# cmbant/getdist

Hardware: AMD Instinct MI355X
Metric: 2D KDE densities/sec (triangle, 50 params, 1e+07 samples) (higher is better)
Workload: dtype f64

## Files before the change

getdist_amd/_lib.py:

```python

import ctypes as C
import os
import subprocess

import numpy as np

_HERE = os.path.dirname(os.path.abspath(__file__))
LIB_PATH = os.path.join(_HERE, "csrc", "libgdhip.so")

GD_OK, GD_ERR_BADARG, GD_ERR_NOMEM, GD_ERR_HIP, GD_ERR_EMPTY, GD_ERR_SOLVER, GD_ERR_FFT, GD_ERR_NODEVICE, GD_ERR_TIMEOUT = \
    0, -1, -2, -3, -4, -5, -6, -7, -8


class GdhipError(RuntimeError):
    def __init__(self, code, msg):
        super().__init__("libgdhip error %d: %s" % (code, msg))
        self.code = code


class GdhipTimeout(GdhipError):
    """GD_ERR_TIMEOUT: a collective or the communicator set-up gave up waiting for a peer; the library has aborted and dropped
    the communicator, so the ranks renegotiate over the host application's own channel (parallel.init_library_comm)."""


def build_native(force=False):
    script = os.path.join(_HERE, "csrc", "build.sh")
    if force:
        for f in os.listdir(os.path.join(_HERE, "csrc")):
            if f.endswith(".o") or f.endswith(".so"):
                os.remove(os.path.join(_HERE, "csrc", f))
    subprocess.run(["bash", script], check=True)
    return LIB_PATH


_p = C.c_void_p
_i32, _i64, _f64 = C.c_int32, C.c_int64, C.c_double
_pd = C.POINTER(C.c_double)
_pi32 = C.POINTER(C.c_int32)
_pi64 = C.POINTER(C.c_int64)

SIGNATURES = {
    "gd_device_count": (C.c_int, []),
    "gd_create": (C.c_int, [C.c_int, C.POINTER(_p)]),
    "gd_destroy": (None, [_p]),
    "gd_last_error": (C.c_char_p, [_p]),
    "gd_version": (C.c_char_p, []),
    "gd_device_info": (C.c_int, [_p, _pi64]),
    "gd_sync": (C.c_int, [_p]),
    "gd_dev_alloc": (C.c_int, [_p, _i64, C.POINTER(_p)]),
    "gd_dev_free": (C.c_int, [_p, _p]),
    "gd_memcpy_h2d": (C.c_int, [_p, _p, _p, _i64]),
    "gd_memcpy_d2h": (C.c_int, [_p, _p, _p, _i64]),
    "gd_memcpy_d2h_async": (C.c_int, [_p, _p, _p, _i64]),
    "gd_copy_sync": (C.c_int, [_p]),
    "gd_memcpy_d2d": (C.c_int, [_p, _p, _p, _i64]),
    "gd_memset": (C.c_int, [_p, _p, C.c_int, _i64]),
    "gd_gather_items": (C.c_int, [_p, _p, _p, _pi32, _i32, _i64]),
    "gd_host_alloc": (C.c_int, [_p, _i64, C.POINTER(_p)]),
    "gd_host_free": (C.c_int, [_p, _p]),
    "gd_kde_lag_sums_2d": (C.c_int, [_p, _i32, _i32, _pd, _pi64, _i32, _pd]),
    "gd_autocov_lags_batch": (C.c_int, [_p, _pi32, _i32, _pd, _i64, _i32, _pd]),
    "gd_kde_lag_sums_batch": (C.c_int, [_p, _pi32, _i32, _pd, _pi64, _i32, _pd]),
    "gd_autocov_lags_range_batch": (C.c_int, [_p, _pi32, _i32, _pd, _i64, _i64, _i64, _i32, _pd]),
    "gd_timer_start": (C.c_int, [_p]),
    "gd_timer_stop_ms": (C.c_int, [_p, _pd]),
    "gd_upload": (C.c_int, [_p, _p, _i64, _i64, _i64, _i64, _p]),
    "gd_num_rows": (C.c_int, [_p, _pi64, _pi64]),
    "gd_column_ptr": (C.c_int, [_p, _i64, C.POINTER(_p)]),
    "gd_weight_stats": (C.c_int, [_p, _i64, _i64, _f64, _pd]),
    "gd_col_stats": (C.c_int, [_p, _i64, _i64, _pd]),
    "gd_cov": (C.c_int, [_p, _pi32, _i32, _i64, _i64, _pd, _pd, _pd, _pd]),
    "gd_quantiles": (C.c_int, [_p, _pi32, _i32, _i64, _i64, _pd, _i32, _pd]),
    "gd_quantiles_mm_probe": (C.c_int, [_p, _pi32, _i32, _i64, _i64, _pd, _i32, _pd, _pd, _pd, _pd, C.POINTER(C.c_int32)]),
    "gd_quantiles_mm": (C.c_int, [_p, _pi32, _i32, _i64, _i64, _pd, _i32, _pd, _pd]),
    "gd_autocov_lags": (C.c_int, [_p, _i32, _f64, _i64, _i32, _pd]),
    "gd_kde_lag_sums": (C.c_int, [_p, _i32, _f64, _pi64, _i32, _pd]),
    "gd_hist1d": (C.c_int, [_p, _pi32, _i32, _pd, _pd, _i32, _pd]),
    "gd_hist1d_dev": (C.c_int, [_p, _pi32, _i32, _pd, _pd, _i32, _p]),
    "gd_bin_indices": (C.c_int, [_p, _i32, _f64, _f64, _i32, _i32, _pi32, _pi64]),
    "gd_prebin": (C.c_int, [_p, _i32, _f64, _f64, _i32, _p]),
    "gd_prebin_batch": (C.c_int, [_p, _pi32, _i32, _pd, _pd, _i32, C.POINTER(_p)]),
    "gd_prebin8_batch": (C.c_int, [_p, _pi32, _i32, _pd, _pd, _i32, C.POINTER(_p), _pi64]),
    "gd_hist2d_prebinned8": (C.c_int, [_p, _i32, C.POINTER(_p), C.POINTER(_p), _p]),
    "gd_prebin8_hist2d": (C.c_int, [_p, _pi32, _i32, _pd, _pd, C.POINTER(_p), _pi64, _i32, C.POINTER(_p), C.POINTER(_p), _p]),
    "gd_hist2d": (C.c_int, [_p, _i32, _pi32, _pi32, _pd, _pd, _pd, _pd, _i32, _p]),
    "gd_hist2d_prebinned": (C.c_int, [_p, _i32, C.POINTER(_p), C.POINTER(_p), _i32, _p]),
    "gd_minmax_affine": (C.c_int, [_p, _i32, _pi32, _pi32, _pd, _pd, _pd]),
    "gd_hist2d_sheared": (C.c_int, [_p, _i32, _pi32, _pi32, _pd, _pd, _pd, _pd, _pd, _pd, _i32, _p]),
    "gd_dct1d": (C.c_int, [_p, _i32, _i32, _pd, _pd]),
    "gd_isj1d": (C.c_int, [_p, _i32, _i32, _pd, _pd, _pd, _pi32]),
    "gd_isj1d_dev": (C.c_int, [_p, _i32, _i32, _p, _pd, _pd, _pi32]),
    "gd_density1d": (C.c_int, [_p, _i32, _i32, _pd, _pd, _pi32, _pi32, _i32, _i32, _pd, _pi32]),
    "gd_density1d_dev": (C.c_int, [_p, _i32, _i32, _p, _pd, _pi32, _pi32, _i32, _i32, _pd, _pi32]),
    "gd_density1d_batch": (C.c_int, [_p, _p, _p, _i32, _pi32, _i32, _pd, _pd, _pd]),
    "gd_kopt2d": (C.c_int, [_p, _i32, _i32, _p, _pd, _pi32, _pd, _pd, _pd]),
    "gd_kopt2d_enqueue": (C.c_int, [_p, _i32, _i32, _p, _pd, _pi32, _pd, _pd, _p, _pi32]),
    "gd_kopt2d_finish": (C.c_int, [_p, _p, _i32, _i32, _p, _pd]),
    "gd_get_h": (C.c_int, [_p, _i32, _pd, _pd, _pd, _pi32, _pd]),
    "gd_density2d": (C.c_int, [_p, _i32, _i32, _p, _pd, _pd, _pd, _pi32, _pi32, _i32, _i32, _p, _pi32]),
    "gd_copy_mark": (C.c_int, [_p, _pi32]),
    "gd_copy_wait": (C.c_int, [_p, _i32]),
    "gd_density2d_enqueue": (C.c_int, [_p, _i32, _i32, _p, _pd, _pd, _pd, _pi32, _pi32, _i32, _i32, _p, _p]),
    "gd_density2d_enqueue_indexed": (C.c_int, [_p, _i32, _i32, _p, _pi32, _pd, _pd, _pd, _pi32, _pi32, _i32, _i32, _p, _p]),
    "gd_attach_samples": (C.c_int, [_p, _p]),
    "gd_bind_thread": (C.c_int, [_p]),
    "gd_contour_levels": (C.c_int, [_p, _i32, _i32, _p, _pd, _i32, _pd, _pi32]),
    "gd_limits1d": (C.c_int, [_p, _i32, _i32, _pd, _pd, _pd, _pd, _i32, _i32, _pd, _pi32]),
    "gd_set_extra_column": (C.c_int, [_p, _i32, _pd]),
    "gd_aux_weights": (C.c_int, [_p, _pd]),
    "gd_col_minmax": (C.c_int, [_p, _pi32, _i32, _i64, _i64, _i32, C.c_double, _pd]),
    "gd_weights_integral": (C.c_int, [_p, _pi32]),
    "gd_thin_rows": (C.c_int, [_p, _i64, _i64, _i64, _i32, _p, _i64, C.POINTER(C.c_int64)]),
    "gd_binary_transitions": (C.c_int, [_p, _pi32, _i32, _p, _i64, _pd, _i32, C.POINTER(C.c_int64)]),
    "gd_thinned_lag_sums": (C.c_int, [_p, _pi32, _i32, _pd, _p, _i64, _i32, _pd]),
    "gd_density2d_masked": (C.c_int, [_p, _i32, _p, C.c_double, C.c_double, C.c_double, _i32, _i32, _i32, _i32, _pd, _pd,
                                      C.POINTER(C.c_ubyte), _p, _pi32]),
    "gd_like_weights": (C.c_int, [_p, _pd, _i32, C.c_double, _pd]),
    "gd_select_weights": (C.c_int, [_p, _i32]),
    "gd_likes1d": (C.c_int, [_p, _i32, _i32, _pd, _pd, _pd, _pd, _pi32, _pi32, _i32, _pd, _pi32]),
    "gd_likes2d": (C.c_int, [_p, _i32, _i32, _p, _p, _pd, _pd, _pd, _pi32, _pi32, _i32, _p, _pi32]),
    "gd_circ_convolve": (C.c_int, [_p, _i32, _i32, _pd, _pd, _pd]),
    "gd_convolve1d_direct": (C.c_int, [_p, _pd, _i64, _pd, _i64, _pd]),
    "gd_autoconvolve": (C.c_int, [_p, _i32, _f64, _i32, _pd, _i64, _i64, _i64, _i32, _pd]),
    "gd_like_stats": (C.c_int, [_p, _i32, _pd]),
    "gd_batch2d_grid_sizes": (C.c_int, [_p, _i32, _pd, _pi32, _i32, _pi32]),
    "gd_density2d_batch": (C.c_int, [_p, _p, _p, _p, _i32, _pd, _pd, _pd, _pi32, _i32, _p, _p, _p, _i64, _pi32, _pd, _pd, _pi32,
                                     _pi32]),
    "gd_comm_unique_id": (C.c_int, [_p]),
    "gd_comm_init": (C.c_int, [_p, _i32, _i32, _p]),
    "gd_comm_info": (C.c_int, [_p, _pi32, _pi32]),
    "gd_comm_destroy": (C.c_int, [_p]),
    "gd_comm_abandon": (C.c_int, [_p]),
    "gd_comm_allgather": (C.c_int, [_p, _pd, _i64, _pd]),
    "gd_comm_allreduce_sum": (C.c_int, [_p, _pd, _i64]),
    "gd_comm_allgather_dev": (C.c_int, [_p, _p, _i64, _p]),
    "gd_comm_allreduce_sum_dev": (C.c_int, [_p, _p, _i64, _p]),
    "gd_batch2d_finish": (C.c_int, [_p]),
    "gd_batch2d_invalidate": (C.c_int, [_p]),
    "gd_batch2d_exchanges": (C.c_int, [_p, C.POINTER(C.c_int64)]),
    "gd_comm_rccl_path": (C.c_int, [C.c_char_p, C.c_int32, C.POINTER(C.c_int32)]),
    "gd_upload_shard": (C.c_int, [_p, _p, _i64, _i64, _i64, _i64, _i64, _p]),
    "gd_comm_share_columns": (C.c_int, [_p, C.POINTER(C.c_int64)]),
    "gd_histnd_batch": (C.c_int, [_p, _i32, _pi32, _pi32, _pd, _pd, _i32, _i32, _i32, _pd, _pd, _pd]),
    "gd_pca_corr": (C.c_int, [_p, _pi32, _i32, _pi32, _pd, _pd, _pd]),
    "gd_pca_project": (C.c_int, [_p, _pi32, _i32, _pi32, _pd, _pd, _pd, _i32, _i32, _pd, _pd, _pd, _pd, _pd, _pd]),
    "gd_mixture_nll": (C.c_int, [_p, _pi32, _i32, _i32, _pd, _pd, _pd, _i64, _i64, _pd]),
}

GD_HISTND_MAXD, GD_HISTND_MAX_BINS = 25, 1 << 25
GD_HISTND_H, GD_HISTND_LIKES, GD_HISTND_LMIN = 1, 2, 4
GD_PCA_MAX_PROJ = 448

_lib = None


def load_library():
    global _lib
    if _lib is None:
        if not os.path.exists(LIB_PATH):
            raise ImportError("libgdhip.so is not built: run `python -c 'import __graft_entry__ as g; g.build()'` "
                              "or getdist_amd/csrc/build.sh (there is no CPU fallback)")
        lib = C.CDLL(LIB_PATH)
        for name, (res, args) in SIGNATURES.items():
            fn = getattr(lib, name)
            fn.restype = res
            fn.argtypes = args
        _lib = lib
    return _lib


def _dp(a):
    return a.ctypes.data_as(_pd)


def _ip(a):
    return a.ctypes.data_as(_pi32)


def _f64arr(a):
    return np.ascontiguousarray(a, dtype=np.float64)


def _i32arr(a):
    return np.ascontiguousarray(a, dtype=np.int32)


class DevBuf:

    def __init__(self, ctx, nbytes):
        self.ctx = ctx
        self.nbytes = int(nbytes)
        self.ptr, self.capacity = ctx._take_block(self.nbytes)

    def free(self):
        if self.ptr and self.ctx.h:
            self.ctx._give_block(self.ptr, self.capacity)
        self.ptr = None

    def __del__(self):
        try:
            self.free()
        except Exception:
            pass

    def to_host(self, shape, dtype=np.float64, offset_bytes=0, pinned=False):
        out = self.ctx.pinned_array(shape, dtype) if pinned else np.empty(shape, dtype=dtype)
        self.ctx._check(self.ctx.lib.gd_memcpy_d2h(self.ctx.h, out.ctypes.data, self.ptr + offset_bytes, out.nbytes))
        return out

    def to_host_async(self, shape, dtype=np.float64):
        out = self.ctx.pinned_array(shape, dtype)
        self.ctx._check(self.ctx.lib.gd_memcpy_d2h_async(self.ctx.h, out.ctypes.data, self.ptr, out.nbytes))
        return out

    def from_host(self, arr, offset_bytes=0):
        arr = np.ascontiguousarray(arr)
        self.ctx._check(self.ctx.lib.gd_memcpy_h2d(self.ctx.h, self.ptr + offset_bytes, arr.ctypes.data, arr.nbytes))


class Context:

    def __init__(self, device=0):
        self.lib = load_library()
        self.h = None
        if self.lib.gd_device_count() <= 0:
            raise RuntimeError("getdist_amd needs a HIP device (no CPU fallback): none visible")
        h = _p()
        rc = self.lib.gd_create(int(device), C.byref(h))
        if rc != 0:
            raise GdhipError(rc, "gd_create(device=%d) failed" % device)
        self.h = h
        self.device = device
        self.N = self.n = 0
        self.weighted = False
        self._pinned = []
        self._free_blocks = []
        self._pinned_blocks = []
        self.comm_world = self.comm_rank = 0

    PINNED_POOL_LIMIT = 8 << 30

    def pinned_array(self, shape, dtype=np.float64):
        import sys

        nbytes = int(np.prod(shape)) * np.dtype(dtype).itemsize
        best = None
        for k, (ptr, nb, buf) in enumerate(self._pinned):
            if nb >= nbytes and sys.getrefcount(buf) <= 3 and (best is None or nb < self._pinned[best][1]):
                best = k
        if best is None:
# ... 482 lines not shown
                                                   thresholds.shape[1], out.ctypes.data_as(C.POINTER(C.c_int64))))
        return out

    def thinned_lag_sums(self, cols, means, rows, K, maxoff):
        cols, means = _i32arr(cols), _f64arr(means)
        out = np.zeros((len(cols), int(maxoff)))
        self._check(self.lib.gd_thinned_lag_sums(self.h, _ip(cols), len(cols), _dp(means), rows.ptr, int(K), int(maxoff),
                                                 _dp(out)))
        return out

    def like_weights(self, loglikes, mode, mean_loglike):
        if loglikes is None:
            self._check(self.lib.gd_like_weights(self.h, None, 0, 0.0, None))
            return None
        ll = _f64arr(loglikes)
        if ll.shape != (self.N,):
            raise ValueError("loglikes must have one entry per sample row")
        tot = C.c_double()
        self._check(self.lib.gd_like_weights(self.h, _dp(ll), int(mode), float(mean_loglike), C.byref(tot)))
        return tot.value

    def select_weights(self, which):
        self._check(self.lib.gd_select_weights(self.h, int(which)))

    def likes1d(self, hist, likehist, P, smooth, winw, flags, shade_mean_loglikes):
        hist, likehist, P = _f64arr(hist), _f64arr(likehist), _f64arr(P)
        B, F = hist.shape
        smooth, winw, flags = _f64arr(smooth), _i32arr(winw), _i32arr(flags)
        out = np.zeros_like(hist)
        status = np.zeros(B, dtype=np.int32)
        self._check(self.lib.gd_likes1d(self.h, B, F, _dp(hist), _dp(likehist), _dp(P), _dp(smooth), _ip(winw),
                                        _ip(flags), int(bool(shade_mean_loglikes)), _dp(out), _ip(status)))
        return out, status

    def likes2d(self, d_hist, d_likehist, B, F, rx, ry, corr, winw, flags, mbc):
        out = self.alloc(B * F * F * 8)
        rx, ry, corr, winw, flags = _f64arr(rx), _f64arr(ry), _f64arr(corr), _i32arr(winw), _i32arr(flags)
        status = np.zeros(B, dtype=np.int32)
        self._check(self.lib.gd_likes2d(self.h, B, F, d_hist.ptr, d_likehist.ptr, _dp(rx), _dp(ry), _dp(corr),
                                        _ip(winw), _ip(flags), int(mbc), out.ptr, _ip(status)))
        return out, status

    def circ_convolve(self, a, b):
        a, b = _f64arr(a), _f64arr(b)
        if a.shape != b.shape or a.ndim not in (1, 2):
            raise ValueError("circ_convolve needs two arrays of one shape, one- or two-dimensional")
        n0, n1 = (1, a.shape[0]) if a.ndim == 1 else a.shape
        out = np.empty_like(a)
        self._check(self.lib.gd_circ_convolve(self.h, int(n0), int(n1), _dp(a), _dp(b), _dp(out)))
        return out

    def convolve1d_direct(self, x, y):
        x, y = _f64arr(x), _f64arr(y)
        out = np.empty(x.size + y.size - 1)
        self._check(self.lib.gd_convolve1d_direct(self.h, _dp(x), x.size, _dp(y), y.size, _dp(out)))
        return out

    def autoconvolve(self, s, n, normalize=True, x=None, col=-1, mean=0.0, use_weights=False):
        out = np.empty(int(n))
        xx = None if x is None else _f64arr(x)
        self._check(self.lib.gd_autoconvolve(self.h, int(col), float(mean), int(bool(use_weights)),
                                             None if xx is None else _dp(xx), 0 if xx is None else xx.size, int(s), int(n),
                                             int(bool(normalize)), _dp(out)))
        return out

    def like_stats(self, col):
        out = np.zeros(8)
        self._check(self.lib.gd_like_stats(self.h, int(col), _dp(out)))
        return dict(min=out[0], max=out[1], norm=out[2], sum_wl=out[3], sum_wl2=out[4], sum_w_exp_plus=out[5],
                    sum_w_exp_minus=out[6], argmin=int(out[7]))

    def batch2d_grid_sizes(self, settings, n, corr, pairs32):
        F = np.zeros(len(pairs32), dtype=np.int32)
        rc = self.lib.gd_batch2d_grid_sizes(C.byref(settings), int(n), _dp(corr), _ip(pairs32), len(pairs32), _ip(F))
        if rc != 0:
            raise GdhipError(rc, "gd_batch2d_grid_sizes: bad argument")
        return F

    def density2d_batch(self, twin, settings, params, n, corr, cov, lag_probe, pairs32, exchange, grids, status, meta, levels,
                        level_status):
        tokens = np.full(2, -1, dtype=np.int32)
        self._check(self.lib.gd_density2d_batch(
            self.h, None if twin is None else twin.h, C.byref(settings), C.cast(params, _p), int(n), _dp(corr), _dp(cov),
            None if lag_probe is None else _dp(lag_probe), _ip(pairs32), len(pairs32),
            None if exchange is None else C.cast(exchange, _p), None, grids.ctypes.data, int(grids.size),
            status.ctypes.data_as(_pi32), _dp(meta), None if levels is None else _dp(levels),
            None if level_status is None else _ip(level_status), _ip(tokens)))
        return int(tokens[0]), int(tokens[1])

    @staticmethod
    def comm_unique_id():
        buf = C.create_string_buffer(128)
        rc = load_library().gd_comm_unique_id(buf)
        if rc != 0:
            raise GdhipError(rc, "gd_comm_unique_id failed (librccl.so missing?)")
        return buf.raw

    def comm_init(self, world, rank, id128):
        self._check(self.lib.gd_comm_init(self.h, int(world), int(rank), C.create_string_buffer(bytes(id128), 128)))
        self.comm_world, self.comm_rank = int(world), int(rank)

    def comm_allgather(self, vec):
        v = _f64arr(vec).ravel()
        out = np.empty((self.comm_world, v.size))
        self._check(self.lib.gd_comm_allgather(self.h, _dp(v), v.size, _dp(out)))
        return out

    def comm_allreduce_sum(self, vec):
        v = _f64arr(vec).ravel().copy()
        self._check(self.lib.gd_comm_allreduce_sum(self.h, _dp(v), v.size))
        return v

    def comm_destroy(self):
        self._check(self.lib.gd_comm_destroy(self.h))
        self.comm_world = 0

    def comm_info(self):
        wd, rk = C.c_int32(0), C.c_int32(0)
        self._check(self.lib.gd_comm_info(self.h, C.byref(wd), C.byref(rk)))
        return int(wd.value), int(rk.value)

    def comm_abandon(self):
        if self.h is not None:
            self.lib.gd_comm_abandon(self.h)

    def density1d_batch(self, settings, params, n, cols32, want_hist=False):
        cols32 = _i32arr(cols32)
        B, F = len(cols32), int(settings.fine_bins)
        P = np.zeros((B, F))
        hist = np.zeros((B, F)) if want_hist else None
        meta = np.zeros((B, 9))
        self._check(self.lib.gd_density1d_batch(self.h, C.byref(settings), C.cast(params, _p), int(n), _ip(cols32), B, _dp(P),
                                                None if hist is None else _dp(hist), _dp(meta)))
        return P, hist, meta

    def batch2d_finish(self):
        self._check(self.lib.gd_batch2d_finish(self.h))

    def batch2d_invalidate(self):
        self._check(self.lib.gd_batch2d_invalidate(self.h))

    def batch2d_exchanges(self):
        c = C.c_int64(0)
        self._check(self.lib.gd_batch2d_exchanges(self.h, C.byref(c)))
        return int(c.value)

    def kopt2d(self, d_hist, B, F, neff, do_corr, fallback_t, corr):
        neff, do_corr, fallback_t, corr = _f64arr(neff), _i32arr(do_corr), _f64arr(fallback_t), _f64arr(corr)
        out = np.zeros((B, 12))
        self._check(self.lib.gd_kopt2d(self.h, B, F, d_hist.ptr if isinstance(d_hist, DevBuf) else d_hist, _dp(neff),
                                       _ip(do_corr), _dp(fallback_t), _dp(corr), _dp(out)))
        return out

    def get_h(self, psi, neff, corr, do_corr):
        psi, neff, corr, do_corr = _f64arr(psi).reshape(-1, 6), _f64arr(neff), _f64arr(corr), _i32arr(do_corr)
        out = np.zeros((len(psi), 4))
        self._check(self.lib.gd_get_h(self.h, len(psi), _dp(psi), _dp(neff), _dp(corr), _ip(do_corr), _dp(out)))
        return out

    def density2d(self, d_hist, B, F, rx, ry, corr, winw, flags, bco, mbc, out=None):
        out = out or self.alloc(B * F * F * 8)
        rx, ry, corr, winw, flags = _f64arr(rx), _f64arr(ry), _f64arr(corr), _i32arr(winw), _i32arr(flags)
        status = np.zeros(B, dtype=np.int32)
        self._check(self.lib.gd_density2d(self.h, B, F, d_hist.ptr if isinstance(d_hist, DevBuf) else d_hist, _dp(rx),
                                          _dp(ry), _dp(corr), _ip(winw), _ip(flags), int(bco), int(mbc), out.ptr,
                                          _ip(status)))
        return out, status
```

getdist_amd/csrc/batch2d.hip:

```cpp
#include "batch1d.hpp"
#include "batch2d.hpp"
#include "ctx.hpp"

namespace {

gd_ctx* C(void* h) { return (gd_ctx*)h; }

const gdb::Ops kOps = {
     [](void* h) { return gd_bind_thread(C(h)); },
     [](void* h, int64_t* N, int64_t* n) { return gd_num_rows(C(h), N, n); },
    [](void* h, int32_t* hw) {
        gd_ctx* c = C(h);
        *hw = c->w == nullptr ? 0 : ((!c->w8 && !c->w_integral && c->w_sum > 1e-200 && c->w_sum < 1e200) ? 2 : 1);
        return 0;
    },
     [](void* h, int64_t bytes, void** out) { return gd_dev_alloc(C(h), bytes, out); },
     [](void* h, void* p) { return gd_dev_free(C(h), p); },
    [](void* h, const int32_t* cols, int32_t ncols, const double* binmin, const double* width, int32_t F, void* const* d_idx,
       int64_t* bad) { return gd_prebin8_batch(C(h), cols, ncols, binmin, width, F, d_idx, bad); },
    [](void* h, int32_t B, const void* const* ix, const void* const* iy, void* d_hist) {
        return gd_hist2d_prebinned8(C(h), B, ix, iy, d_hist);
    },
    [](void* h, const int32_t* cols, int32_t ncols, const double* binmin, const double* width, void* const* d_idx, int64_t* bad,
       int32_t B, const void* const* ix, const void* const* iy, void* d_hist) {
        return gd_prebin8_hist2d(C(h), cols, ncols, binmin, width, d_idx, bad, B, ix, iy, d_hist);
    },
    [](void* h, int32_t col, double binmin, double width, int32_t F, void* d_idx) {
        return gd_prebin(C(h), col, binmin, width, F, d_idx);
    },
    [](void* h, int32_t B, const void* const* ix, const void* const* iy, int32_t F, void* d_hist) {
        return gd_hist2d_prebinned(C(h), B, ix, iy, F, d_hist);
    },
    [](void* h, int32_t B, const int32_t* ci, const int32_t* cj, const double* a, const double* b, double* out) {
        return gd_minmax_affine(C(h), B, ci, cj, a, b, out);
    },
    [](void* h, int32_t B, const int32_t* ci, const int32_t* cj, const double* r0, const double* r1, const double* xmin,
       const double* dx, const double* ymin, const double* dy, int32_t F, void* d_hist) {
        return gd_hist2d_sheared(C(h), B, ci, cj, r0, r1, xmin, dx, ymin, dy, F, d_hist);
    },
    [](void* h, int32_t B, int32_t F, const void* d_hist, const double* neff, const int32_t* do_corr, const double* fallback_t,
       const double* corr, double* out) { return gd_kopt2d(C(h), B, F, d_hist, neff, do_corr, fallback_t, corr, out); },
    [](void* h, void* d_dst, int64_t dst_first, const void* d_src, const int32_t* index, int32_t count, int64_t item_bytes) {
        return gd_gather_items(C(h), (char*)d_dst + dst_first * item_bytes, d_src, index, count, item_bytes);
    },
    [](void* h, int32_t B, int32_t F, const void* d_hist, const int32_t* hist_index, const double* rx, const double* ry,
       const double* corr, const int32_t* winw, const int32_t* flags, int32_t bco, int32_t mbc, void* d_P, int32_t* status_pinned) {
        return gd_density2d_enqueue_indexed(C(h), B, F, d_hist, hist_index, rx, ry, corr, winw, flags, bco, mbc, d_P, status_pinned);
    },
     [](void* h, void* dst, const void* d_src, int64_t bytes) { return gd_memcpy_d2h_async(C(h), dst, d_src, bytes); },
     [](void* h, int32_t* token) { return gd_copy_mark(C(h), token); },
    [](void* h, int32_t token) {
        if (!gd_ctx_alive(C(h))) return 0;
        const int rc = gd_copy_wait(C(h), token);
        return rc == GD_ERR_BADARG ? 0 : rc;
    },
     [](void* h) { return gd_ctx_alive(C(h)) ? gd_copy_sync(C(h)) : 0; },
    [](void* h, int32_t B, int32_t F, const void* d_P, const double* contours, int32_t nc, double* out, int32_t* status) {
        return gd_contour_levels(C(h), B, F, d_P, contours, nc, out, status);
    },
    [](void* h, const int32_t* cols, int32_t ncols, const double* means, int64_t k0, int32_t nlags, double* out) {
        return gd_autocov_lags_batch(C(h), cols, ncols, means, k0, nlags, out);
    },
    [](void* h, const int32_t* cols, int32_t ncols, const double* inv4s2, const int64_t* lags, int32_t nlags, double* out) {
        return gd_kde_lag_sums_batch(C(h), cols, ncols, inv4s2, lags, nlags, out);
    },
    [](void* h, int32_t col, double inv4s2, const int64_t* lags, int32_t nlags, double* out) {
        return gd_kde_lag_sums(C(h), col, inv4s2, lags, nlags, out);
    },
     [](void* h) { return gd_last_error(C(h)); },
    [](void* h, void** aux) {
        gd_ctx* a = nullptr;
        int rc = gd_create(C(h)->device, &a);
        if (rc == 0) rc = gd_attach_samples(a, C(h));
        if (rc == 0) rc = gd_stream_priority(a, 1);
        if (rc) {
            if (a) gd_destroy(a);
            return gd_fail(C(h), rc, "could not create the third context of a batched call");
        }
        *aux = a;
        return 0;
    },
    [](void* aux) {
        gd_destroy(C(aux));
        return 0;
    },
    [](void* h, int32_t B, int32_t F, const void* d_hist, const double* neff, const int32_t* do_corr, const double* fallback_t,
       const double* corr, void* d_rows, int32_t* ticket) {
        return gd_kopt2d_enqueue(C(h), B, F, d_hist, neff, do_corr, fallback_t, corr, d_rows, ticket);
    },
    [](void* h, void* stage_a_h, int32_t ticket, int32_t B, void* d_rows, double* out) {
        return gd_kopt2d_finish(C(h), C(stage_a_h), ticket, B, d_rows, out);
    },
     [](void* h) { return C(h)->comm ? C(h)->comm_world : 0; },
     [](void* h, double* inout, int64_t count) { return gd_comm_allreduce_sum(C(h), inout, count); },
     [](void* ctx, int level) { return gd_stream_priority(C(ctx), level); },
    [](void* h, const int32_t* cols, int32_t ncols, const double* binmin, const double* width, int32_t F, void* const* d_idx) {
        return gd_prebin_batch(C(h), cols, ncols, binmin, width, F, d_idx);
    },
};

const gdb::Ops1D kOps1D = {
    [](void* h, const int32_t* cols, int32_t ncols, const double* binmin, const double* width, int32_t F, void* d_hist) {
        return gd_hist1d_dev(C(h), cols, ncols, binmin, width, F, d_hist);
    },
    [](void* h, int32_t B, int32_t F, const void* d_hist, const double* neff, double* hfrac, int32_t* status) {
        return gd_isj1d_dev(C(h), B, F, d_hist, neff, hfrac, status);
    },
    [](void* h, int32_t B, int32_t F, const void* d_hist, const double* smooth, const int32_t* winw, const int32_t* flags,
       int32_t bco, int32_t mbc, double* P_out, int32_t* status) {
        return gd_density1d_dev(C(h), B, F, d_hist, smooth, winw, flags, bco, mbc, P_out, status);
    },
    [](void* h, void* dst, const void* d_src, int64_t bytes) {
        const int rc = gd_fetch(C(h), dst, d_src, (size_t)bytes);
        return rc ? rc : gd_stream_sync(C(h));
    },
};

void release_state(gd_ctx* ctx, bool destroy) {
    gdb::State* st = (gdb::State*)ctx->batch_state;
    if (!st) return;
    gdb::release_all(*st, kOps, ctx);
    if (destroy) {
        delete st;
        ctx->batch_state = nullptr;
    }
}

gdb::State& state_of(gd_ctx* ctx) {
    if (!ctx->batch_state) {
        ctx->batch_state = new gdb::State();
        ctx->batch_state_release = release_state;
    }
    return *(gdb::State*)ctx->batch_state;
}

}

extern "C" {

int gd_batch2d_grid_sizes(const gd_batch2d_settings* settings, int32_t n, const double* corr, const int32_t* pairs, int32_t P,
                          int32_t* F_out) {
    if (!settings || !corr || (!pairs && P > 0) || (!F_out && P > 0) || n <= 0 || P < 0) return GD_ERR_BADARG;
    for (int k = 0; k < 2 * P; ++k)
        if (pairs[k] < 0 || pairs[k] >= n) return GD_ERR_BADARG;
    gdb::PairScalars ps;
    gdb::pair_scalars(*settings, n, corr, pairs, P, ps);
    for (int k = 0; k < P; ++k) F_out[k] = ps.F[k];
    return GD_OK;
}

int gd_density2d_batch(gd_ctx* ctx, gd_ctx* twin, const gd_batch2d_settings* settings, gd_param2d* params, int32_t n,
                       const double* corr, const double* cov, const double* lag_probe, const int32_t* pairs, int32_t P,
                       gd_neff_exchange_fn exchange, void* exchange_user, void* grids_pinned, int64_t grids_doubles,
                       int32_t* status_pinned, double* meta, double* levels, int32_t* level_status, int32_t* tokens_out2) {
    GD_REQUIRE(ctx && settings && params && corr && cov && tokens_out2 && n > 0 && P >= 0, "bad argument");
    GD_REQUIRE(P == 0 || (pairs && grids_pinned && status_pinned && meta), "bad argument");
    GD_REQUIRE(ctx->cols, "no samples uploaded");
    GD_REQUIRE(!twin || (twin != ctx && twin->cols == ctx->cols), "the second context must be attached to the first (gd_attach_samples)");
    GD_REQUIRE(ctx->w_sel == 0, "auxiliary weights are selected");
    GD_REQUIRE(!settings->want_levels || (settings->contours && settings->ncontours > 0 && levels && level_status), "contour levels requested without room for them");
    GD_HIP(hipSetDevice(ctx->device));
    int rc;
    try {
        gdb::Call call(state_of(ctx), kOps, ctx, twin, *settings, params, n, corr, cov, lag_probe, pairs, P, exchange, exchange_user,
                       (double*)grids_pinned, grids_doubles, status_pinned, meta, levels, level_status);
        rc = call.run(tokens_out2);
        if (rc) ctx->err = call.err;
    } catch (const std::exception& e) {
        rc = gd_fail(ctx, GD_ERR_NOMEM, "gd_density2d_batch: %s", e.what());
    }
    return rc;
}

int gd_density1d_batch(gd_ctx* ctx, const gd_density1d_settings* settings, gd_param2d* params, int32_t n, const int32_t* cols,
                       int32_t B, double* P_out, double* hist_out, double* meta) {
    GD_REQUIRE(ctx && settings && params && cols && P_out && meta && n > 0 && B > 0, "bad argument");
    GD_REQUIRE(ctx->cols, "no samples uploaded");
    GD_REQUIRE(ctx->w_sel == 0, "auxiliary weights are selected");
    GD_HIP(hipSetDevice(ctx->device));
    int rc;
    try {
        std::string err;
        rc = gdb::density1d_batch(state_of(ctx), kOps, kOps1D, ctx, *settings, params, n, cols, B, P_out, hist_out, meta, &err);
        if (rc) ctx->err = err;
    } catch (const std::exception& e) {
        rc = gd_fail(ctx, GD_ERR_NOMEM, "gd_density1d_batch: %s", e.what());
    }
    return rc;
}

int gd_batch2d_finish(gd_ctx* ctx) {
    GD_REQUIRE(ctx, "null context");
    if (!ctx->batch_state) return GD_OK;
    GD_HIP(hipSetDevice(ctx->device));
    return gdb::finish_all(*(gdb::State*)ctx->batch_state, kOps, ctx);
}

int gd_batch2d_exchanges(gd_ctx* ctx, int64_t* count_out) {
    GD_REQUIRE(ctx && count_out, "null argument");
    *count_out = 0;
    if (ctx->batch_state) {
        gdb::State& st = *(gdb::State*)ctx->batch_state;
        std::lock_guard<std::mutex> g(st.mu);
        *count_out = st.exchanges_entered;
    }
    return GD_OK;
}

int gd_batch2d_invalidate(gd_ctx* ctx) {
    GD_REQUIRE(ctx, "null context");
    if (!ctx->batch_state) return GD_OK;
    gdb::invalidate_index_columns(*(gdb::State*)ctx->batch_state);
    return GD_OK;
}

}
```

getdist_amd/csrc/batch2d.hpp:

```cpp
#pragma once
#include <math.h>
#include <stdint.h>
#include <stdio.h>
#include <stdlib.h>
#include <string.h>
#include <time.h>

#include <algorithm>
#include <atomic>
#include <chrono>
#include <condition_variable>
#include <deque>
#include <functional>
#include <future>
#include <map>
#include <mutex>
#include <string>
#include <thread>
#include <vector>

#include "../../include/gdhip.h"

namespace gdb {

struct Ops {
    int (*bind_thread)(void* h);
    int (*num_rows)(void* h, int64_t* N, int64_t* n);
    int (*weights_kind)(void* h, int32_t* has_weights);
    int (*dev_alloc)(void* h, int64_t bytes, void** out);
    int (*dev_free)(void* h, void* p);
    int (*prebin8_batch)(void* h, const int32_t* cols, int32_t ncols, const double* binmin, const double* width, int32_t F,
                         void* const* d_idx, int64_t* bad);
    int (*hist2d_prebinned8)(void* h, int32_t B, const void* const* ix, const void* const* iy, void* d_hist);
    int (*prebin8_hist2d)(void* h, const int32_t* cols, int32_t ncols, const double* binmin, const double* width,
                          void* const* d_idx, int64_t* bad, int32_t B, const void* const* ix, const void* const* iy, void* d_hist);
    int (*prebin)(void* h, int32_t col, double binmin, double width, int32_t F, void* d_idx);
    int (*hist2d_prebinned)(void* h, int32_t B, const void* const* ix, const void* const* iy, int32_t F, void* d_hist);
    int (*minmax_affine)(void* h, int32_t B, const int32_t* ci, const int32_t* cj, const double* a, const double* b, double* out);
    int (*hist2d_sheared)(void* h, int32_t B, const int32_t* ci, const int32_t* cj, const double* r0, const double* r1,
                          const double* xmin, const double* dx, const double* ymin, const double* dy, int32_t F, void* d_hist);
    int (*kopt2d)(void* h, int32_t B, int32_t F, const void* d_hist, const double* neff, const int32_t* do_corr,
                  const double* fallback_t, const double* corr, double* out);
    int (*gather_items)(void* h, void* d_dst, int64_t dst_first, const void* d_src, const int32_t* index, int32_t count,
                        int64_t item_bytes);
    int (*density2d_enqueue)(void* h, int32_t B, int32_t F, const void* d_hist, const int32_t* hist_index, const double* rx,
                             const double* ry, const double* corr, const int32_t* winw, const int32_t* flags, int32_t bco,
                             int32_t mbc, void* d_P, int32_t* status_pinned);
    int (*d2h_async)(void* h, void* dst, const void* d_src, int64_t bytes);
    int (*copy_mark)(void* h, int32_t* token);
    int (*copy_wait)(void* h, int32_t token);
    int (*copy_sync)(void* h);
    int (*contour_levels)(void* h, int32_t B, int32_t F, const void* d_P, const double* contours, int32_t nc, double* out,
                          int32_t* status);
    int (*autocov_lags_batch)(void* h, const int32_t* cols, int32_t ncols, const double* means, int64_t k0, int32_t nlags,
                              double* out);
    int (*kde_lag_sums_batch)(void* h, const int32_t* cols, int32_t ncols, const double* inv4s2, const int64_t* lags,
                              int32_t nlags, double* out);
    int (*kde_lag_sums)(void* h, int32_t col, double inv4s2, const int64_t* lags, int32_t nlags, double* out);
    const char* (*last_error)(void* h);
    int (*create_aux)(void* h, void** aux);
    int (*destroy_aux)(void* aux);
    int (*kopt2d_enqueue)(void* h, int32_t B, int32_t F, const void* d_hist, const double* neff, const int32_t* do_corr,
                          const double* fallback_t, const double* corr, void* d_rows, int32_t* ticket);
    int (*kopt2d_finish)(void* h, void* stage_a_h, int32_t ticket, int32_t B, void* d_rows, double* out);
    int (*comm_world)(void* h);
    int (*comm_allreduce_sum)(void* h, double* inout, int64_t count);
    int (*stream_priority)(void* ctx, int level);
    int (*prebin_batch)(void* h, const int32_t* cols, int32_t ncols, const double* binmin, const double* width, int32_t F,
                        void* const* d_idx);
};

static inline double py_pow(double x, double y) {
    volatile double e = y;
    return pow(x, e);
}
static inline double np_minimum(double a, double b) { return (a < b || isnan(a)) ? a : b; }
static inline double np_maximum(double a, double b) { return (a > b || isnan(a)) ? a : b; }
static inline double np_sign(double x) { return isnan(x) ? x : (x > 0 ? 1.0 : (x < 0 ? -1.0 : 0.0)); }

static inline int frame_size(int n) {
    long long best = 1LL << 40;
    const int odd[5] = {1, 3, 5, 9, 15};
    for (int a = 4; a < 28; ++a)
        for (int q = 0; q < 5; ++q) {
            const long long v = (1LL << a) * odd[q];
            if (v >= n && v < best) best = v;
        }
    return (int)best;
}

static inline bool chol_shear(double c00, double c10, double c11, double S[4], double r[2]) {
    if (!(c00 > 0)) return false;
    const double l00 = sqrt(c00);
    const double l10 = c10 * (1.0 / l00);
    const double d = c11 - l10 * l10;
    if (!(d > 0)) return false;
    const double l11 = sqrt(d);
    double i00, i10, i11;
    if (fabs(l10) > fabs(l00)) {
        const double l = l00 * (1.0 / l10);
        const double u11 = 0.0 - l * l11;
        i10 = 1.0 * (1.0 / u11);
        i00 = (0.0 - l11 * i10) * (1.0 / l10);
        i11 = (0.0 - l * 1.0) * (1.0 / u11);
    } else {
        const double l = l10 * (1.0 / l00);
        i00 = 1.0 * (1.0 / l00);
        i10 = (0.0 - l * 1.0) * (1.0 / l11);
        i11 = 1.0 * (1.0 / l11);
    }
    S[0] = l00 * i00, S[1] = 0.0 * i00, S[2] = l10 * i00, S[3] = l11 * i00;
    r[0] = i10 / i00, r[1] = i11 / i00;
    return true;
}

struct PairScalars {
    std::vector<int32_t> jx, jy, F, warn;
    std::vector<int64_t> nbin2D;
    std::vector<double> actual, corr;
};

static inline void pair_scalars(const gd_batch2d_settings& s, int n, const double* corrmat, const int32_t* pairs, int P,
                                PairScalars& ps) {
    ps.jx.resize(P), ps.jy.resize(P), ps.F.resize(P), ps.warn.assign(P, 0), ps.nbin2D.resize(P), ps.actual.resize(P),
        ps.corr.resize(P);
    const int base_F = s.fine_bins_2D;
    for (int k = 0; k < P; ++k) {
        const int a = pairs[2 * k], b = pairs[2 * k + 1];
        ps.jx[k] = a, ps.jy[k] = b;
        const double actual = corrmat[(size_t)b * n + a];
        double c = actual;
        if (fabs(fabs(c) - 1.0) <= 1e-8) {
            ps.warn[k] |= 1;
            c = np_sign(c) * s.max_corr_2D;
        }
        if (fabs(c) < 0.1) c = 0.0;
        const double m = np_minimum(s.max_corr_2D, fabs(c));
        const double angle_scale = np_maximum(0.2, sqrt(1 - m * m));
        ps.nbin2D[k] = (int64_t)nearbyint((double)s.num_bins_2D / angle_scale);
        const int64_t scaled = 192 * (int64_t)(3 / angle_scale) / 3;
        ps.F[k] = (c != 0 && base_F < scaled && (int64_t)(1 / angle_scale) > 1) ? (int32_t)scaled : base_F;
        ps.actual[k] = actual, ps.corr[k] = c;
    }
}

static inline void bin_edges(const gd_param2d& p, double* binmin, double* binmax) {
    const double border = (p.range_max - p.range_min) * 0.1;
    double lo = np_minimum(p.param_min, p.range_min);
    if (!p.has_limits_bot) lo = lo - border;
    double hi = np_maximum(p.param_max, p.range_max);
    if (!p.has_limits_top) hi = hi + border;
    *binmin = lo, *binmax = hi;
}

struct NeffInput {
    int64_t N;
    double norm, sum_w2;
};

static inline int neff_from_lags(const NeffInput& in, int64_t maxoff, double min_corr, const double* sums, int nseed_tail,
                                 const std::function<int(int64_t, double*)>& lag_sum, double* neff_out) {
    const int64_t N = in.N;
    if (maxoff > N / 10) maxoff = N / 10;
    const int64_t uncorr_len = N / 2;
    int64_t nav = 0;
    for (int64_t k = uncorr_len; k < uncorr_len + 5; ++k) nav += N - k;
    double s5 = 0.0;
    for (int q = 0; q < 5; ++q) s5 += sums[q];
    const double uncorr_term = s5 / (double)nav;
    const double n = (double)N;
    std::map<int64_t, double> cache;
    for (int q = 0; q < nseed_tail; ++q) cache[q + 1] = sums[5 + q];
    int rc = 0;
    auto corr_k = [&](int64_t k) -> double {
        auto it = cache.find(k);
        double v;
        if (it == cache.end()) {
            v = NAN;
            const int e = lag_sum(k, &v);
            if (e) rc = e;
            cache[k] = v;
        } else {
            v = it->second;
        }
        return v - (n - (double)k) * uncorr_term;
    };
    const double corr0 = in.sum_w2;
    const double threshold = min_corr * corr0;
    const double c1 = corr_k(1);
    double Nn;
    if (c1 < threshold) {
        Nn = corr0;
    } else {
        const double c2 = corr_k(2);
        if (c2 > threshold) {
            int64_t max_k = maxoff;
            while (max_k > 10) {
                if (corr_k(max_k / 3) >= threshold) break;
                max_k /= 3;
            }
            const int64_t step_size = max_k < 20 ? 1 : max_k / 10;
            double cum_sum = c1 + c2;
            for (int64_t k = 3; k < maxoff + 1; k += step_size) {
                const double test_val = corr_k(k);
                if (test_val < threshold) break;
                cum_sum += k > 3 ? test_val * (double)step_size : (test_val * (double)step_size) / 2;
            }
            Nn = corr0 + 2 * cum_sum;
        } else {
            Nn = corr0 + 2 * c1;
        }
    }
    if (rc) return rc;
    *neff_out = py_pow(in.norm, 2.0) / Nn;
    return 0;
}

struct Plan {
    std::vector<int8_t> branch;
    std::vector<uint8_t> has_limits;
    std::vector<double> rangex, rangey, ratio, neff, fallback_t;
    std::vector<int32_t> si, sj;
    std::vector<uint8_t> swap, has_imin, has_imax;
    std::vector<double> imin, imax, S, r;
// ... 51 lines not shown
    void* ptr = nullptr;
    double binmin = NAN, width = NAN;
    bool valid = false;
};

struct Pending {
    std::vector<void*> blocks;
    int32_t tok_main = -1, tok_twin = -1;
    void* twin = nullptr;
    bool live = false;
};

struct State {
    std::mutex mu;
    std::vector<std::pair<void*, int64_t>> free_blocks;
    std::map<void*, int64_t> capacity;
    int64_t cached_bytes = 0;
    std::map<std::tuple<int, int, int>, IdxCol> idx;
    Pending prev;
    void* aux = nullptr;
    void* aux2 = nullptr;
    int64_t exchanges_entered = 0;
    static constexpr int64_t kCacheLimit = 16LL << 30;
};

struct Pool {
    State& st;
    const Ops& ops;
    void* h;
    void* take(int64_t bytes, int* rc) {
        {
            std::lock_guard<std::mutex> g(st.mu);
            int best = -1;
            for (size_t k = 0; k < st.free_blocks.size(); ++k) {
                const int64_t cap = st.free_blocks[k].second;
                if (cap >= bytes && cap <= 2 * bytes + (1 << 20) && (best < 0 || cap < st.free_blocks[best].second)) best = (int)k;
            }
            if (best >= 0) {
                void* p = st.free_blocks[best].first;
                st.cached_bytes -= st.free_blocks[best].second;
                st.free_blocks.erase(st.free_blocks.begin() + best);
                return p;
            }
        }
        void* p = nullptr;
        int e = ops.dev_alloc(h, bytes, &p);
        if (e == GD_ERR_NOMEM) {
            drop_cached();
            e = ops.dev_alloc(h, bytes, &p);
        }
        if (e) {
            *rc = e;
            return nullptr;
        }
        std::lock_guard<std::mutex> g(st.mu);
        st.capacity[p] = bytes;
        return p;
    }
    void give(void* p) {
        if (!p) return;
        std::unique_lock<std::mutex> g(st.mu);
        const int64_t cap = st.capacity[p];
        if (st.cached_bytes + cap > State::kCacheLimit) {
            st.capacity.erase(p);
            g.unlock();
            ops.dev_free(h, p);
            return;
        }
        st.free_blocks.emplace_back(p, cap);
        st.cached_bytes += cap;
    }
    void drop_cached() {
        std::vector<std::pair<void*, int64_t>> blocks;
        {
            std::lock_guard<std::mutex> g(st.mu);
            blocks.swap(st.free_blocks);
            st.cached_bytes = 0;
            for (auto& b : blocks) st.capacity.erase(b.first);
        }
        for (auto& b : blocks) ops.dev_free(h, b.first);
    }
};

static inline int complete_pending(State& st, const Ops& ops, void* h, Pending& pd) {
    if (!pd.live) return 0;
    int rc = 0;
    if (pd.tok_main >= 0) rc = ops.copy_wait(h, pd.tok_main);
    if (!rc && pd.twin && pd.tok_twin >= 0) rc = ops.copy_wait(pd.twin, pd.tok_twin);
    Pool pool{st, ops, h};
    for (void* p : pd.blocks) pool.give(p);
    pd.blocks.clear();
    pd.live = false;
    return rc;
}

static inline int finish_all(State& st, const Ops& ops, void* h) { return complete_pending(st, ops, h, st.prev); }

static inline void invalidate_index_columns(State& st) {
    std::lock_guard<std::mutex> g(st.mu);
    for (auto& kv : st.idx) kv.second.valid = false;
}

static inline void release_all(State& st, const Ops& ops, void* h) {
    finish_all(st, ops, h);
    Pool pool{st, ops, h};
    {
        std::lock_guard<std::mutex> g(st.mu);
        for (auto& kv : st.idx)
            if (kv.second.ptr) st.free_blocks.emplace_back(kv.second.ptr, st.capacity[kv.second.ptr]);
        st.idx.clear();
    }
    pool.drop_cached();
    if (st.aux) {
        ops.destroy_aux(st.aux);
        st.aux = nullptr;
    }
    if (st.aux2) {
        ops.destroy_aux(st.aux2);
        st.aux2 = nullptr;
    }
}

struct Call {
    State& st;
    const Ops& ops;
    void* h;
    void* twin;
    const gd_batch2d_settings& s;
    gd_param2d* par;
    int n;
    const double* corrmat;
    const double* cov;
    const double* lag_probe;
    const int32_t* pairs;
    int P;
    gd_neff_exchange_fn exchange;
    void* exchange_user;
    double* grids;
    int64_t grids_doubles;
    int32_t* status_pinned;
    double* meta;
    double* levels;
    int32_t* level_status;
    std::string err;

    Call(State& st_, const Ops& ops_, void* h_, void* twin_, const gd_batch2d_settings& s_, gd_param2d* par_, int n_,
         const double* corr_, const double* cov_, const double* lag_probe_, const int32_t* pairs_, int P_,
         gd_neff_exchange_fn ex_, void* ex_user_, double* grids_, int64_t grids_doubles_, int32_t* status_, double* meta_,
         double* levels_, int32_t* level_status_)
        : st(st_), ops(ops_), h(h_), twin(twin_), s(s_), par(par_), n(n_), corrmat(corr_), cov(cov_), lag_probe(lag_probe_),
          pairs(pairs_), P(P_), exchange(ex_), exchange_user(ex_user_), grids(grids_), grids_doubles(grids_doubles_),
          status_pinned(status_), meta(meta_), levels(levels_), level_status(level_status_), pool{st_, ops_, h_} {}

    int64_t N = 0;
    bool unit_weights = true;
    Pool pool;
    PairScalars ps;
    std::vector<int> used;
    std::vector<double> bmin, bmax;
    std::vector<double> fwx, fwy;
    std::vector<int> F_list;
    std::map<int, std::vector<int>> classes;
    std::map<int, void*> hists;
    Plan plan;
    struct Shear {
        void* d_rot = nullptr;
        std::vector<int> A;
        std::vector<double> r1s, r2s;
    } shear;
    bool have_shear = false;
    bool byte_index_weights = false;
    std::vector<double> rx, ry, cc, smooth, W;
    std::vector<int64_t> winw;
    std::vector<int32_t> flags, group;
    std::vector<void*> call_blocks;
    std::vector<void*> bin_stale;
    std::mutex enq_mu;
    std::atomic<int> bin_launching{0};
    bool hold_neff_for_binning = false;
    std::atomic<int> bin_done{0};
    bool shear_after_binning = false;
    std::future<int> shear_future;
    bool shear_deferred = false;
    std::atomic<bool> shear_joined{true};
    std::mutex shear_mu;
    std::atomic<int> shear_hist_state{1};
    int shear_hist_rc = 0;
    std::atomic<int> first_part_done{0};
    static constexpr int32_t kStatusPending = 0x7fffffff;
    std::atomic<const volatile int32_t*> first_part_flag{nullptr};
    int reports_enqueued = 0;
    std::shared_future<int> bin_future;
    std::mutex bin_mu;
    std::atomic<int> bins_first_done{0};
    int bins_first_rows = 0;
    int bin_rc = 0;
    bool bin_joined = true;
    int join_binning() {
        std::lock_guard<std::mutex> g(bin_mu);
        if (!bin_joined) {
            bin_joined = true;
            bin_rc = bin_future.valid() ? bin_future.get() : 0;
            mark("binning: joined");
        }
        return bin_rc;
    }
    size_t base_part_size(size_t total, int F) const {
        size_t want = 2;
        if (const char* e = getenv("GDHIP_KOPT_PARTS")) want = (size_t)std::max(1, atoi(e));
        size_t part = std::max<size_t>((size_t)s_kopt_split_min(), (total + want - 1) / want);
        size_t align = 256;
        if (const char* e = getenv("GDHIP_KOPT_PART_ALIGN")) align = (size_t)std::max(0, atoi(e));
        if (align > 1 && F == 256 && part > align) part = std::max<size_t>(align, (part + align / 2 - 1) / align * align);
        return part;
    }
    static size_t first_part_size(size_t part) {
        if (const char* e = getenv("GDHIP_KOPT_FIRST_PART")) {
            const size_t f = (size_t)std::max(0, atoi(e));
            if (f > 0 && f < part) return f;
        }
        return part;
    }
    static int shear_hold_us() {
        const char* e = getenv("GDHIP_BATCH_SHEAR_HOLD_US");
        return e ? atoi(e) : 0;
    }
    int join_shear(bool release = false) {
        if (release) first_part_done.store(1);
        std::lock_guard<std::mutex> g(shear_mu);
        if (shear_joined.load()) return 0;
        const int e = shear_future.valid() ? shear_future.get() : 0;
        shear_joined.store(true);
        mark("shear: joined");
        return e;
    }
    int64_t grid_off = 0;
    int status_at = 0;
    int batch_no = 0;
    std::vector<void*> conv_ctxs;
    std::vector<int> side_classes;
    std::vector<int> order;

    std::mutex tl_mu;
    std::vector<std::pair<double, std::string>> tl;
    bool tl_on = getenv("GDHIP_BATCH_LOG") != nullptr;
    static double now_ms() {
        timespec ts;
        clock_gettime(CLOCK_MONOTONIC, &ts);
        return ts.tv_sec * 1e3 + ts.tv_nsec * 1e-6;
    }
    void mark(const char* what, int a = -1, int b = -1) {
        if (!tl_on) return;
        char buf[160];
        if (a >= 0 && b >= 0)
            snprintf(buf, sizeof buf, "%s (%d, %d)", what, a, b);
        else if (a >= 0)
            snprintf(buf, sizeof buf, "%s (%d)", what, a);
        else
            snprintf(buf, sizeof buf, "%s", what);
        std::lock_guard<std::mutex> g(tl_mu);
        tl.emplace_back(now_ms(), buf);
    }
    void dump_timeline() {
        if (!tl_on || tl.empty()) return;
        std::sort(tl.begin(), tl.end());
        fprintf(stderr, "---- gd_density2d_batch host timeline (ms)\n");
        for (auto& e : tl) fprintf(stderr, "%9.3f  %s\n", e.first - tl[0].first, e.second.c_str());
    }

    std::mutex err_mu;
    int fail(int code, const std::string& msg) {
        std::lock_guard<std::mutex> g(err_mu);
        if (err.empty()) err = msg;
        return code;
    }
    int dev_fail(int code, void* ctx) {
        const char* m = ops.last_error(ctx);
        return fail(code, m && *m ? m : "device call failed");
    }
#define GDB_DEV(ctx_, call_)                       \
    do {                                           \
        const int rc__ = (call_);                  \
        if (rc__) return dev_fail(rc__, (ctx_));   \
    } while (0)
#define GDB_TRY(call_)            \
    do {                          \
        const int rc__ = (call_); \
        if (rc__) return rc__;    \
    } while (0)

    double* M(int k) { return meta + (size_t)k * GD_BATCH2D_META; }

    int neff_batch(const std::vector<int>& js, bool owned_only, double min_corr = 0.05) {
        std::vector<int32_t> todo;
        for (int j : js)
            if (isnan(par[j].neff) && (!owned_only || (par[j].owned & 1))) todo.push_back(j);
        if (todo.empty()) return 0;
        mark("neff: start", (int)todo.size());
        if (s.uncorrelated_sampler) {
            for (int j : todo) par[j].neff = py_pow(s.norm, 2.0) / s.sum_w2;
            return 0;
        }
        const int m = (int)todo.size();
        const int64_t max_off = N / 10;
        const int nl = (int)std::min<int64_t>(8, max_off + 1);
        std::vector<double> lag0((size_t)m * nl);
        bool have = lag_probe != nullptr && nl == 8;
        if (have)
            for (int row = 0; row < m && have; ++row)
                for (int k = 0; k < nl; ++k) {
                    lag0[(size_t)row * nl + k] = lag_probe[(size_t)todo[row] * 8 + k];
                    if (isnan(lag0[(size_t)row * nl + k])) have = false;
                }
        if (!have) {
            std::vector<double> means(m);
            for (int row = 0; row < m; ++row) means[row] = par[todo[row]].mean;
            GDB_DEV(h, ops.autocov_lags_batch(h, todo.data(), m, means.data(), 0, nl, lag0.data()));
        }
        std::vector<double> kstd(m), inv4s2(m);
        std::vector<int64_t> maxoffs(m);
        bool all_uncorrelated_at_lag_1 = true;
        for (int row = 0; row < m; ++row) {
            const gd_param2d& p = par[todo[row]];
            double c[8];
            for (int k = 0; k < nl; ++k) c[k] = lag0[(size_t)row * nl + k] / (double)(N - k) / p.var;
            int first_below = -1;
            for (int k = 0; k < nl; ++k)
                if (!(c[k] > min_corr * c[0])) {
                    first_below = k;
// ... 53 lines not shown
    int neff_exchange(bool* exchanged) {
        if (exchange && !*exchanged) {
            *exchanged = true;
            std::vector<double> v(n);
            for (int j = 0; j < n; ++j) v[j] = par[j].neff;
            if (exchange(exchange_user, v.data(), n)) return fail(GD_ERR_HIP, "N_eff exchange failed");
            for (int j = 0; j < n; ++j)
                if (isnan(par[j].neff)) par[j].neff = v[j];
        } else if (!exchange && s.comm_exchange && !*exchanged) {
            *exchanged = true;
            if (!ops.comm_world || ops.comm_world(h) < 1) return fail(GD_ERR_BADARG, "comm_exchange without a communicator (gd_comm_init)");
            {
                std::lock_guard<std::mutex> g(st.mu);
                ++st.exchanges_entered;
            }
            std::vector<double> v(n, 0.0);
            for (int j = 0; j < n; ++j)
                if ((par[j].owned & 1) && !isnan(par[j].neff)) v[j] = par[j].neff;
            GDB_DEV(h, ops.comm_allreduce_sum(h, v.data(), n));
            for (int j = 0; j < n; ++j)
                if (isnan(par[j].neff) && v[j] > 0) par[j].neff = v[j];
        }
        return 0;
    }
    int neff_complete(bool* exchanged) {
        const int rc = neff_exchange(exchanged);
        if (rc || s.pair_neff) return rc;
        return neff_batch(used, false);
    }

    int index_column16(void* ctx, int j, int F, void** out) {
        const double fw = (bmax[j] - bmin[j]) / (F - 1);
        IdxCol c;
        {
            std::lock_guard<std::mutex> g(st.mu);
            c = st.idx[std::make_tuple(j, F, 2)];
        }
        if (!(c.valid && c.binmin == bmin[j] && c.width == fw)) {
            if (!c.ptr) {
                int rc = 0;
                c.ptr = pool.take(N * 2 + 64, &rc);
                if (!c.ptr) return dev_fail(rc, h);
            }
            GDB_DEV(ctx, ops.prebin(ctx, j, bmin[j], fw, F, c.ptr));
            c.binmin = bmin[j], c.width = fw, c.valid = true;
            std::lock_guard<std::mutex> g(st.mu);
            st.idx[std::make_tuple(j, F, 2)] = c;
        }
        *out = c.ptr;
        return 0;
    }

    int index_columns16(void* ctx, const std::vector<int>& cols, int F) {
        if (!ops.prebin_batch) return 0;
        std::vector<int32_t> todo;
        std::vector<double> b0, w;
        std::vector<void*> bufs;
        for (int j : cols) {
            const double fw = (bmax[j] - bmin[j]) / (F - 1);
            IdxCol c;
            {
                std::lock_guard<std::mutex> g(st.mu);
                c = st.idx[std::make_tuple(j, F, 2)];
            }
            if (c.valid && c.binmin == bmin[j] && c.width == fw) continue;
            if (!c.ptr) {
                int rc = 0;
                c.ptr = pool.take(N * 2 + 64, &rc);
                if (!c.ptr) return dev_fail(rc, h);
                std::lock_guard<std::mutex> g(st.mu);
                st.idx[std::make_tuple(j, F, 2)] = c;
            }
            todo.push_back(j), b0.push_back(bmin[j]), w.push_back(fw), bufs.push_back(c.ptr);
        }
        if (todo.size() < 2) return 0;
        GDB_DEV(ctx, ops.prebin_batch(ctx, todo.data(), (int)todo.size(), b0.data(), w.data(), F, bufs.data()));
        std::lock_guard<std::mutex> g(st.mu);
        for (size_t q = 0; q < todo.size(); ++q) {
            IdxCol& c = st.idx[std::make_tuple((int)todo[q], F, 2)];
            c.binmin = b0[q], c.width = w[q], c.valid = true;
        }
        return 0;
    }

    int main_class() const {
        int best = F_list.empty() ? 0 : F_list[0];
        for (int F : F_list)
            if (classes.at(F).size() > classes.at(best).size()) best = F;
        return best;
    }
    int binning(void* ctx, int part = 0) {
        const int main_F = main_class();
        for (int F : F_list) {
            if ((part == 1 && F != main_F) || (part == 2 && F == main_F)) continue;
            const std::vector<int>& members = classes.at(F);
            const int B = (int)members.size();
            int rc = 0;
            if (F == 256 && (unit_weights || byte_index_weights) && B >= 64) {
                std::vector<int> cols;
                std::vector<char> seen(n, 0);
                for (int k : members)
                    if (!seen[ps.jx[k]]) seen[ps.jx[k]] = 1, cols.push_back(ps.jx[k]);
                for (int k : members)
                    if (!seen[ps.jy[k]]) seen[ps.jy[k]] = 1, cols.push_back(ps.jy[k]);
                std::vector<int32_t> todo;
                std::vector<double> b0, w;
                std::vector<void*> bufs;
                {
                    std::lock_guard<std::mutex> g(st.mu);
                    for (int j : cols) {
                        const double fw = (bmax[j] - bmin[j]) / 255;
                        IdxCol& c = st.idx[std::make_tuple(j, 256, 1)];
                        if (c.valid && c.binmin == bmin[j] && c.width == fw) continue;
                        todo.push_back(j), b0.push_back(bmin[j]), w.push_back(fw), bufs.push_back(c.ptr);
                    }
                }
                for (size_t q = 0; q < todo.size(); ++q)
                    if (!bufs[q]) {
                        bufs[q] = pool.take(N + 64, &rc);
                        if (!bufs[q]) return dev_fail(rc, h);
                        std::lock_guard<std::mutex> g(st.mu);
                        IdxCol& c = st.idx[std::make_tuple((int)todo[q], 256, 1)];
                        c.ptr = bufs[q], c.valid = false;
                    }
                std::vector<const void*> ix(B), iy(B);
                {
                    std::lock_guard<std::mutex> g(st.mu);
                    for (int q = 0; q < B; ++q) {
                        ix[q] = st.idx[std::make_tuple((int)ps.jx[members[q]], 256, 1)].ptr;
                        iy[q] = st.idx[std::make_tuple((int)ps.jy[members[q]], 256, 1)].ptr;
                    }
                }
                void* d = pool.take((int64_t)B * 65536 * 8, &rc);
                if (!d) return dev_fail(rc, h);
                std::vector<int64_t> bad(todo.size() + 1, 0);
                mark("binning: prebin8 + hist2d launch", (int)todo.size(), B);
                bin_launching.store(1);
                const int B1 = (F == main_F && bins_first_rows > 0 && bins_first_rows < B) ? bins_first_rows : B;
                int e = ops.prebin8_hist2d(ctx, todo.data(), (int)todo.size(), b0.data(), w.data(), bufs.data(), bad.data(), B1,
                                           ix.data(), iy.data(), d);
                mark("binning: prebin8 + hist2d done", B1);
                if (e == 0 || e == GD_ERR_SOLVER) {
                    std::lock_guard<std::mutex> g(st.mu);
                    for (size_t q = 0; q < todo.size(); ++q) {
                        IdxCol& c = st.idx[std::make_tuple((int)todo[q], 256, 1)];
                        c.binmin = b0[q], c.width = w[q], c.valid = bad[q] == 0;
                    }
                }
                bool published = false;
                if (e == 0 && B1 < B) {
                    {
                        std::lock_guard<std::mutex> g(enq_mu);
                        hists[F] = d;
                    }
                    published = true;
                    bins_first_done.store(1);
                    e = ops.hist2d_prebinned8(ctx, B - B1, ix.data() + B1, iy.data() + B1, (char*)d + (int64_t)B1 * 65536 * 8);
                    mark("binning: the other rows done", B - B1);
                    if (e == 0) continue;
                }
                if (e == 0) {
                    std::lock_guard<std::mutex> g(enq_mu);
                    hists[F] = d;
                    continue;
                }
                if (published) {
                    std::lock_guard<std::mutex> g(enq_mu);
                    hists.erase(F);
                    bin_stale.push_back(d);
                } else {
                    pool.give(d);
                }
                if (e != GD_ERR_SOLVER) return dev_fail(e, ctx);
            }
            bin_launching.store(1);
            {
                std::vector<int> cols;
                std::vector<char> seen(n, 0);
                for (int k : members) {
                    if (!seen[ps.jx[k]]) seen[ps.jx[k]] = 1, cols.push_back(ps.jx[k]);
                    if (!seen[ps.jy[k]]) seen[ps.jy[k]] = 1, cols.push_back(ps.jy[k]);
                }
                GDB_TRY(index_columns16(ctx, cols, F));
            }
            std::vector<const void*> ix(B), iy(B);
            for (int q = 0; q < B; ++q) {
                void* p;
                GDB_TRY(index_column16(ctx, ps.jx[members[q]], F, &p));
                ix[q] = p;
            }
            for (int q = 0; q < B; ++q) {
                void* p;
                GDB_TRY(index_column16(ctx, ps.jy[members[q]], F, &p));
                iy[q] = p;
            }
            void* d = pool.take((int64_t)B * F * F * 8, &rc);
            if (!d) return dev_fail(rc, h);
            const int e = ops.hist2d_prebinned(ctx, B, ix.data(), iy.data(), F, d);
            mark("binning: hist2d_prebinned done", B, F);
            if (e) {
                pool.give(d);
                return dev_fail(e, ctx);
            }
            std::lock_guard<std::mutex> g(enq_mu);
            hists[F] = d;
        }
        bin_launching.store(1);
        return 0;
    }

    int shear_histograms(void* ctx) {
        const int base_F = s.fine_bins_2D;
        shear.A.clear();
        for (int k = 0; k < P; ++k)
            if (plan.branch[k] == 0) shear.A.push_back(k);
        have_shear = true;
        const int nA = (int)shear.A.size();
        if (!nA) return 0;
        std::vector<int32_t> ci(nA), cj(nA);
        std::vector<double> r0(nA), r1(nA), mm((size_t)2 * nA);
        for (int row = 0; row < nA; ++row) {
            const int k = shear.A[row];
            ci[row] = plan.si[k], cj[row] = plan.sj[k], r0[row] = plan.r[(size_t)2 * k], r1[row] = plan.r[(size_t)2 * k + 1];
        }
        mark("shear: start", nA);
        GDB_DEV(ctx, ops.minmax_affine(ctx, nA, ci.data(), cj.data(), r0.data(), r1.data(), mm.data()));
        mark("shear: minmax done");
        std::vector<double> xmin(nA), dx(nA), ymin(nA), dy(nA);
        shear.r1s.resize(nA), shear.r2s.resize(nA);
        for (int row = 0; row < nA; ++row) {
            const int k = shear.A[row];
            const double mn = par[plan.si[k]].param_min, mx = par[plan.si[k]].param_max;
            const double delta = mx - mn;
            const double rmin = plan.has_imin[k] ? plan.imin[k] : mn - delta * 0.1;
            const double rmax = plan.has_imax[k] ? plan.imax[k] : mx + delta * 0.1;
            const double R1 = rmax - rmin;
            const double mn2 = mm[(size_t)2 * row], mx2 = mm[(size_t)2 * row + 1];
            const double delta2 = mx2 - mn2;
            const double rmin2 = mn2 - delta2 * 0.1;
            const double R2 = (mx2 + delta2 * 0.1) - rmin2;
            xmin[row] = rmin, dx[row] = R1 / (base_F - 1), ymin[row] = rmin2, dy[row] = R2 / (base_F - 1);
            shear.r1s[row] = R1, shear.r2s[row] = R2;
        }
        int rc = 0;
        shear.d_rot = pool.take((int64_t)nA * base_F * base_F * 8, &rc);
        if (!shear.d_rot) return dev_fail(rc, h);
        GDB_DEV(ctx, ops.hist2d_sheared(ctx, nA, ci.data(), cj.data(), r0.data(), r1.data(), xmin.data(), dx.data(), ymin.data(),
                                        dy.data(), base_F, shear.d_rot));
        mark("shear: histograms done");
        return 0;
    }

    void set_scales(const std::vector<int>& ks) {
        const double a = fabs(s.smooth_scale_2D);
        for (int k : ks) {
            rx[k] = W[(size_t)3 * k] * a / fwx[k];
            ry[k] = W[(size_t)3 * k + 1] * a / fwy[k];
            cc[k] = W[(size_t)3 * k + 2];
            finish_scale(k);
        }
    }
    void finish_scale(int k) {
        smooth[k] = np_maximum(rx[k], ry[k]);
        const double w = nearbyint(2.5 * smooth[k]);
        winw[k] = (isfinite(w) && w > 1) ? (int64_t)w : 1;
        if (smooth[k] < 2) ps.warn[k] |= 2;
    }

    struct Batch {
        std::vector<int> pos, ks;
    };
    int class_batches(int F, const std::vector<char>& only, std::vector<Batch>& batches) {
        const std::vector<int>& members = classes.at(F);
        std::vector<int> pos_all;
        for (int q = 0; q < (int)members.size(); ++q)
            if (only.empty() || only[members[q]]) pos_all.push_back(q);
        batches.clear();
        if (pos_all.empty()) return 0;
        int64_t mb = (int64_t)(s_max_batch_bytes() / ((double)F * F * 8 * 30));
        int max_batch = (int)std::max<int64_t>(1, std::min<int64_t>(mb, s_max_batch()));
        const int first_batch = s_first_batch();
        std::vector<int> gorder;
        for (int q : pos_all) {
            const int g = group[members[q]];
            if (std::find(gorder.begin(), gorder.end(), g) == gorder.end()) gorder.push_back(g);
        }
        for (int g : gorder) {
            std::map<int, std::vector<int>> byS;
            for (int q : pos_all) {
                const int k = members[q];
                if (group[k] != g) continue;
                const int64_t w = winw[k];
                if (w < 1 || w > 2 * (int64_t)F) return fail(GD_ERR_BADARG, "bad window half-width");
                byS[frame_size(F + 2 * (int)w)].push_back(q);
            }
            for (auto& kv : byS) {
                const std::vector<int>& cur = kv.second;
                size_t s0 = 0;
                if (batches.empty() && (int)cur.size() > first_batch) {
                    Batch b;
                    b.pos.assign(cur.begin(), cur.begin() + first_batch);
                    batches.push_back(b);
                    s0 = first_batch;
                }
                for (size_t s1 = s0; s1 < cur.size(); s1 += max_batch) {
                    Batch b;
                    b.pos.assign(cur.begin() + s1, cur.begin() + std::min(cur.size(), s1 + (size_t)max_batch));
                    batches.push_back(b);
                }
            }
        }
        for (auto& b : batches)
            for (int q : b.pos) b.ks.push_back(members[q]);
        return 0;
    }
    int s_first_batch() const {
        if (s.first_batch > 0) return s.first_batch;
        const char* e = getenv("GDHIP_BATCH_FIRST_BATCH");
        return e && atoi(e) > 0 ? atoi(e) : 128;
    }
    int s_max_batch() const {
        if (s.max_batch > 0) return s.max_batch;
        const char* e = getenv("GDHIP_BATCH_MAX_BATCH");
        return e && atoi(e) > 0 ? atoi(e) : 320;
    }
    double s_max_batch_bytes() const { return s.max_batch_bytes > 0 ? s.max_batch_bytes : 24e9; }
    int s_two_min() const { return s.two_streams_min > 0 ? s.two_streams_min : 64; }
    int s_two_split() const { return s.two_streams_split > 0 ? s.two_streams_split : 400; }
    int s_kopt_split_min() const { return s.kopt_split_min > 0 ? s.kopt_split_min : 256; }

    bool is_side(int F) const { return std::find(side_classes.begin(), side_classes.end(), F) != side_classes.end(); }

    int enqueue_batch(int F, const Batch& b, void* force_ctx) {
        const std::vector<int>& members = classes.at(F);
        void* bctx;
        if (force_ctx)
            bctx = force_ctx;
        else if (!side_classes.empty() || P > s_two_split())
            bctx = conv_ctxs[is_side(F) && conv_ctxs.size() > 1 ? 1 : 0];
        else
            bctx = conv_ctxs[batch_no % conv_ctxs.size()];
        ++batch_no;
        const int B = (int)b.pos.size();
        const int64_t item = (int64_t)F * F * 8;
        void* d_hist;
        {
            std::lock_guard<std::mutex> g(enq_mu);
            d_hist = hists.at(F);
        }
        int rc = 0;
        bool whole = B == (int)members.size();
        for (int q = 0; q < B && whole; ++q) whole = b.pos[q] == q;
        std::vector<int32_t> hidx(b.pos.begin(), b.pos.end());
        std::vector<double> rxb(B), ryb(B), ccb(B);
        std::vector<int32_t> wb(B), fb(B);
        for (int q = 0; q < B; ++q) {
            const int k = b.ks[q];
            rxb[q] = rx[k], ryb[q] = ry[k], ccb[q] = cc[k], wb[q] = (int32_t)winw[k], fb[q] = flags[k];
        }
        void* d_P = pool.take((int64_t)B * item, &rc);
        if (!d_P) return dev_fail(rc, h);
        call_blocks.push_back(d_P);
        int32_t* status = status_pinned + status_at;
        for (int q = 0; q < B; ++q) status[q] = kStatusPending;
        if (grid_off + (int64_t)B * F * F > grids_doubles) return fail(GD_ERR_BADARG, "grids_pinned is too small");
        mark(bctx == h ? "conv: enqueue on main" : "conv: enqueue on twin", B, F);
        GDB_DEV(bctx, ops.density2d_enqueue(bctx, B, F, d_hist, whole ? nullptr : hidx.data(), rxb.data(), ryb.data(), ccb.data(),
                                            wb.data(), fb.data(), s.boundary_correction_order, s.mult_bias_correction_order, d_P,
                                            status));
        mark("conv: enqueued");
        if (s.want_levels && levels) {
            std::vector<double> lv((size_t)B * s.ncontours);
            std::vector<int32_t> ls(B);
            GDB_DEV(bctx, ops.contour_levels(bctx, B, F, d_P, s.contours, s.ncontours, lv.data(), ls.data()));
            for (int q = 0; q < B; ++q) {
                memcpy(levels + (size_t)b.ks[q] * s.ncontours, &lv[(size_t)q * s.ncontours], sizeof(double) * s.ncontours);
                level_status[b.ks[q]] = ls[q];
            }
        }
        GDB_DEV(bctx, ops.d2h_async(bctx, grids + grid_off, d_P, (int64_t)B * item));
        for (int q = 0; q < B; ++q) {
            double* m = M(b.ks[q]);
            m[1] = (double)(grid_off + (int64_t)q * F * F);
            m[29] = bctx == twin ? 1.0 : 0.0;
            m[30] = (double)(status_at + q);
        }
        grid_off += (int64_t)B * F * F;
        status_at += B;
        return 0;
    }

    int run_class(int F, const std::vector<char>& only, void* force_ctx) {
        std::vector<Batch> batches;
        GDB_TRY(class_batches(F, only, batches));
        for (const Batch& b : batches) GDB_TRY(enqueue_batch(F, b, force_ctx));
        return 0;
    }

    int enqueue_all() {
        std::vector<int> main_, side;
        for (int F : order) (is_side(F) ? side : main_).push_back(F);
        const std::vector<char> all;
        std::vector<Batch> first;
        size_t first_done = 0;
        if (!side.empty() && !main_.empty()) {
            GDB_TRY(class_batches(main_[0], all, first));
            if (!first.empty()) {
                GDB_TRY(enqueue_batch(main_[0], first[0], nullptr));
                first_done = 1;
            }
        }
        for (int F : side) GDB_TRY(run_class(F, all, nullptr));
        for (size_t q = 0; q < main_.size(); ++q) {
            if (q == 0 && !side.empty()) {
                for (size_t b = first_done; b < first.size(); ++b) GDB_TRY(enqueue_batch(main_[0], first[b], nullptr));
                continue;
            }
            GDB_TRY(run_class(main_[q], all, nullptr));
        }
        return 0;
    }

    struct Launch {
        int F = 0;
        std::vector<int> ks;
        int na = 0;
        void* d_hist = nullptr;
        std::vector<int> pos;
        bool whole = false;
        void* d_batch = nullptr;
        bool own = false;
        void* d_rows = nullptr;
        int32_t ticket = -1;
        std::vector<double> ne, fb, ci;
        std::vector<int32_t> dc;
    };
    typedef std::function<int(const std::vector<int>&, int, int)> ChunkFn;

    template <class BufFn>
    int ready_for(Launch& L, const BufFn& class_buffer) {
        if (L.na > 0 && L.d_hist && !shear_joined.load() && !getenv("GDHIP_BATCH_SHEAR_JOIN_WHOLE")) {
            while (shear_hist_state.load(std::memory_order_acquire) == 0) std::this_thread::sleep_for(std::chrono::microseconds(20));
            mark("shear: histograms awaited");
            if (shear_hist_state.load(std::memory_order_acquire) == 2) {
                (void)join_shear();
                return shear_hist_rc ? shear_hist_rc : GD_ERR_HIP;
            }
        } else if (L.na > 0 || !L.d_hist) {
            const int e = join_shear();
            if (e) return e;
            if (!L.d_hist) L.d_hist = class_buffer(L.F);
            if (!L.d_hist) return fail(GD_ERR_BADARG, "a grid-size class has no histograms");
        }
        return 0;
    }

    int build_batch(Launch& L) {
        const int B = (int)L.ks.size(), F = L.F;
        const int64_t item = (int64_t)F * F * 8;
        L.d_batch = L.d_hist, L.own = false;
        if (!L.whole) {
            int rc = 0;
            L.d_batch = pool.take((int64_t)B * item, &rc);
            if (!L.d_batch) return dev_fail(rc, h);
            L.own = true;
            if (L.na) {
                std::vector<int32_t> idx(L.na);
                for (int a = 0; a < L.na; ++a) idx[a] = a;
                GDB_DEV(h, ops.gather_items(h, L.d_batch, 0, shear.d_rot, idx.data(), L.na, item));
            }
            if (!L.pos.empty()) {
                std::vector<int32_t> idx(L.pos.begin(), L.pos.end());
                GDB_DEV(h, ops.gather_items(h, L.d_batch, L.na, L.d_hist, idx.data(), (int)idx.size(), item));
            }
        }
        L.ne.resize(B), L.fb.resize(B), L.ci.resize(B), L.dc.resize(B);
        for (int row = 0; row < B; ++row) {
            const int k = L.ks[row];
            const bool rowA = row < L.na;
            L.ne[row] = plan.neff[k], L.dc[row] = plan.has_limits[k] ? 0 : 1;
            L.fb[row] = rowA ? -1.0 : plan.fallback_t[k];
            L.ci[row] = rowA ? 0.0 : ps.actual[k];
        }
        return 0;
    }

    int absorb_rows(const Launch& L, const std::vector<double>& out) {
        const int B = (int)L.ks.size();
        for (int row = 0; row < B; ++row) {
            const double* o = &out[(size_t)row * 12];
            if (o[7] == 0 && o[11] != 0) return fail(GD_ERR_BADARG, "bias not positive definite");
        }
        for (int row = 0; row < B; ++row) {
            const int k = L.ks[row];
            const double* o = &out[(size_t)row * 12];
            memcpy(M(k) + 6, o, 12 * sizeof(double));
            double hx, hy, c;
            if (row < L.na) {
                const double hxa = o[8] * shear.r1s[row], hya = o[9] * shear.r2s[row], ca = o[10];
                const double* S = &plan.S[(size_t)4 * k];
                const double k00 = hxa * hxa, k01 = hxa * hya * ca, k11 = hya * hya;
                const double t00 = S[0] * k00 + S[1] * k01, t01 = S[0] * k01 + S[1] * k11;
                const double t10 = S[2] * k00 + S[3] * k01, t11 = S[2] * k01 + S[3] * k11;
                const double c00 = t00 * S[0] + t01 * S[1], c01 = t00 * S[2] + t01 * S[3], c11 = t10 * S[2] + t11 * S[3];
                const double sx = sqrt(c00), sy = sqrt(c11);
                hx = plan.swap[k] ? sy : sx, hy = plan.swap[k] ? sx : sy, c = c01 / sqrt(c00 * c11);
            } else {
                hx = o[8] * plan.rangex[k], hy = o[9] * plan.rangey[k], c = o[10];
            }
            if (o[7] != 0) {
                if (s.raise_on_bandwidth_errors) {
                    char buf[200];
                    snprintf(buf, sizeof buf, "2D kernel density bandwidth optimizer failed for pair %d (columns %d, %d). "
                             "Using fallback width: 2D fixed point: no root in [0, 0.1]", k, (int)ps.jx[k], (int)ps.jy[k]);
                    return fail(GD_ERR_SOLVER, buf);
                }
                ps.warn[k] |= 4;
                const double d = py_pow(plan.neff[k], 1.0 / 6);
                hx = par[ps.jx[k]].sigma_range / d, hy = par[ps.jy[k]].sigma_range / d;
                c = std::max(std::min(ps.actual[k], s.max_corr_2D), -s.max_corr_2D);
            }
            W[(size_t)3 * k] = hx, W[(size_t)3 * k + 1] = hy, W[(size_t)3 * k + 2] = c;
        }
        return 0;
    }

    static bool part_on_main(int index, int nparts) { return nparts > 1 && index >= nparts - std::max(1, 2 * nparts / 5); }

    int bandwidth_2d(bool staged, void* aux, const ChunkFn& on_chunk) {
        const int base_F = s.fine_bins_2D;
        const int m = s.mult_bias_correction_order;
        std::vector<double> widen;
        if (m) {
            widen.resize(P);
            const double e = 1.0 / 6 - 1.0 / (2 + 4 * (1 + m));
            for (int k = 0; k < P; ++k) widen[k] = 1.1 * py_pow(plan.neff[k], e);
        }
        if (!have_shear && !shear_deferred) GDB_TRY(shear_histograms(h));
        std::vector<int> A;
        for (int k = 0; k < P; ++k)
            if (plan.branch[k] == 0) A.push_back(k);
        const int nA = (int)A.size();
        auto class_buffer = [&](int F) -> void* {
            std::lock_guard<std::mutex> g(enq_mu);
            auto it = hists.find(F);
            return it == hists.end() ? nullptr : it->second;
        };
        std::vector<int> waiting;
        for (int k = 0; k < P; ++k)
            if (plan.branch[k] == 1) {
                const double c = std::max(std::min(ps.actual[k], s.max_corr_2D), -s.max_corr_2D);
                const double d = py_pow(plan.neff[k], 1.0 / 6);
                W[(size_t)3 * k] = par[ps.jx[k]].sigma_range / d, W[(size_t)3 * k + 1] = par[ps.jy[k]].sigma_range / d, W[(size_t)3 * k + 2] = c;
                waiting.push_back(k);
            }
        std::vector<Launch> launches;
        bool merged = false;
        for (int F : F_list) {
            const std::vector<int>& mem = classes.at(F);
            std::vector<int> pos_C;
            for (int q = 0; q < (int)mem.size(); ++q)
                if (plan.branch[mem[q]] == 2) pos_C.push_back(q);
            if (F == base_F && !pos_C.empty()) {
                const size_t total = pos_C.size() + (size_t)nA;
                size_t part = total;
                if (staged && (int)pos_C.size() >= s_kopt_split_min()) part = base_part_size(total, F);
                const size_t nparts = shear_deferred ? std::max<size_t>(1, (total + part - 1) / part) : 0;
                for (size_t c0 = 0, first = 1, ip = 0; c0 < pos_C.size(); first = 0, ++ip) {
                    Launch L;
                    const bool carries = shear_deferred ? (ip + 1 == nparts || pos_C.size() - c0 <= part) : first != 0;
                    L.F = F, L.na = carries ? nA : 0, L.d_hist = class_buffer(F);
                    const size_t part_q = (ip == 0 && nparts > 1) ? first_part_size(part) : part;
                    size_t take_ = std::min(pos_C.size() - c0, part_q > (size_t)L.na ? part_q - (size_t)L.na : (size_t)1);
                    if (shear_deferred && carries) take_ = pos_C.size() - c0;
                    L.pos.assign(pos_C.begin() + c0, pos_C.begin() + c0 + take_);
                    c0 += take_;
                    L.whole = L.na == 0 && L.pos.size() == mem.size();
                    for (int q = 0; q < L.na; ++q) L.ks.push_back(A[q]);
                    for (int q : L.pos) L.ks.push_back(mem[q]);
                    launches.push_back(std::move(L));
                }
                merged = true;
                continue;
            }
            if (pos_C.empty()) continue;
            Launch L;
            L.F = F, L.na = 0, L.d_hist = class_buffer(F), L.pos = pos_C, L.whole = pos_C.size() == mem.size();
            for (int q : pos_C) L.ks.push_back(mem[q]);
            launches.push_back(std::move(L));
        }
        if (nA && !merged) {
            GDB_TRY(join_shear(true));
            Launch L;
            L.F = base_F, L.na = nA, L.d_hist = shear.d_rot, L.whole = true;
            L.ks = A;
            launches.push_back(std::move(L));
        }
        const int nl = (int)launches.size();
        if (!staged || nl == 0 || launches[0].na > 0 || !launches[0].d_hist) first_part_done.store(1);
        auto report = [&](std::vector<int> ks, int index) -> int {
            if (!waiting.empty()) {
                std::vector<int> all, later;
                for (int k : waiting) ((shear_deferred && ps.F[k] != base_F && index + 1 < nl) ? later : all).push_back(k);
                all.insert(all.end(), ks.begin(), ks.end());
                ks.swap(all);
                waiting.swap(later);
            }
            if (m)
                for (int k : ks) W[(size_t)3 * k] *= widen[k], W[(size_t)3 * k + 1] *= widen[k];
            if (shear_deferred && index + 1 >= nl) {
                const int e = join_shear();
                if (e) return e;
            }
            if (!ks.empty() || index + 1 >= nl) return on_chunk(ks, index, nl);
            return 0;
        };
        int rc = 0;
        auto rows_binned_first = [&](const Launch& L) {
            if (bins_first_rows <= 0 || L.F != base_F || L.na > 0 || !L.d_hist) return false;
            for (int q : L.pos)
                if (q >= bins_first_rows) return false;
            return true;
        };
        auto whole_binning_for = [&](Launch& L) -> int {
            const int e = join_binning();
            if (e) return e;
            if (L.F == base_F && !L.pos.empty())
                if (void* p = class_buffer(L.F)) L.d_hist = p;
            return 0;
        };
        if (!staged || nl == 0) {
            rc = join_binning();
            for (int q = 0; q < nl && !rc; ++q) {
                Launch& L = launches[q];
                const int B = (int)L.ks.size();
                rc = whole_binning_for(L);
                if (!rc) rc = ready_for(L, class_buffer);
                if (!rc) rc = build_batch(L);
                std::vector<double> out((size_t)B * 12);
                if (!rc) {
                    mark("kopt: launch", B, L.F);
                    rc = ops.kopt2d(h, B, L.F, L.d_batch, L.ne.data(), L.dc.data(), L.fb.data(), L.ci.data(), out.data());
                    mark("kopt: done");
                    if (rc) dev_fail(rc, h);
                }
                if (L.own) pool.give(L.d_batch);
                if (!rc) rc = absorb_rows(L, out);
                if (!rc) rc = report(L.ks, q);
            }
            if (!rc && nl == 0) rc = report({}, 0);
        } else {
            std::mutex mu;
            std::condition_variable cv;
            int n_staged = 0;
            bool abort_ = false;
            std::deque<int> handed;
            std::future<int> enqueuer = std::async(std::launch::async, [&]() -> int {
                ops.bind_thread(h);
                int e = 0;
                for (;;) {
                    int q;
                    {
                        std::unique_lock<std::mutex> g(mu);
                        cv.wait(g, [&] { return !handed.empty(); });
                        q = handed.front();
                        handed.pop_front();
                    }
                    if (q < 0) return e;
                    if (e) continue;
                    if (part_on_main(q, nl) || !shear_deferred) {
                        std::unique_lock<std::mutex> g(mu);
                        cv.wait(g, [&] { return n_staged >= nl || abort_; });
                        if (n_staged < nl) {
                            e = GD_ERR_HIP;
                            continue;
                        }
                    }
                    e = join_binning();
                    if (!e) e = report(launches[q].ks, q);
                    if (reports_enqueued++ == 0 && status_at > 0 && !s.results_in_flight && !getenv("GDHIP_BATCH_SHEAR_ON_ENQUEUE"))
                        first_part_flag.store(status_pinned + status_at - 1);
                    first_part_done.store(1);
                }
            });
            std::future<int> finisher = std::async(std::launch::async, [&]() -> int {
                ops.bind_thread(aux);
                int e = 0;
                auto hand = [&](int q) {
                    std::lock_guard<std::mutex> g(mu);
                    handed.push_back(q);
                    cv.notify_all();
                };
                for (int q = 0; q < nl; ++q) {
                    {
                        std::unique_lock<std::mutex> g(mu);
                        cv.wait(g, [&] { return n_staged > q || abort_; });
                        if (n_staged <= q) break;
                    }
                    Launch& L = launches[q];
                    const int B = (int)L.ks.size();
                    std::vector<double> out((size_t)B * 12);
                    if (!e) {
                        e = ops.kopt2d_finish(aux, h, L.ticket, B, L.d_rows, out.data());
                        mark("kopt: part finished", q, B);
                        if (e) dev_fail(e, aux);
                    } else {
                        ops.copy_sync(h);
                    }
                    if (L.own) pool.give(L.d_batch);
                    pool.give(L.d_rows);
                    if (!e) e = absorb_rows(L, out);
                    if (e || getenv("GDHIP_BATCH_SHEAR_AFTER_GET_H")) first_part_done.store(1);
                    if (!e) hand(q);
                }
                first_part_done.store(1);
                hand(-1);
                return e;
            });
            for (int q = 0; q < nl && !rc; ++q) {
                Launch& L = launches[q];
                const int B = (int)L.ks.size();
                if (!(q == 0 && rows_binned_first(L))) rc = whole_binning_for(L);
                if (!rc) rc = ready_for(L, class_buffer);
                if (!rc) rc = build_batch(L);
                if (!rc) {
                    L.d_rows = pool.take((int64_t)B * GD_KOPT_BLOCK_DOUBLES * 8, &rc);
                    if (!L.d_rows) dev_fail(rc, h);
                }
                if (!rc) {
                    mark("kopt: stage A enqueue", q, B);
                    rc = ops.kopt2d_enqueue(h, B, L.F, L.d_batch, L.ne.data(), L.dc.data(), L.fb.data(), L.ci.data(), L.d_rows, &L.ticket);
                    if (rc) dev_fail(rc, h);
                }
                std::lock_guard<std::mutex> g(mu);
                if (rc) {
                    abort_ = true;
                    if (L.own && L.d_batch) ops.copy_sync(h), pool.give(L.d_batch);
                    if (L.d_rows) pool.give(L.d_rows);
                } else {
                    ++n_staged;
                }
                cv.notify_all();
            }
            {
                std::lock_guard<std::mutex> g(mu);
                if (n_staged < nl) abort_ = true;
                cv.notify_all();
            }
            mark("kopt: every stage A enqueued");
            const int e = finisher.get();
            const int e2 = enqueuer.get();
            if (!rc) rc = e;
            if (!rc) rc = e2;
        }
        {
            const int e0 = join_binning();
            const int e = join_shear(true);
            if (!rc) rc = e0;
            if (!rc) rc = e;
        }
        if (shear.d_rot) pool.give(shear.d_rot), shear.d_rot = nullptr;
        return rc;
    }

    int run(int32_t* tokens_out2) {
        tokens_out2[0] = tokens_out2[1] = -1;
        const int base_F = s.fine_bins_2D, bco = s.boundary_correction_order;
        const double ss = s.smooth_scale_2D;
        if (fabs(s.max_corr_2D) > 1) return fail(GD_ERR_BADARG, "max_corr_2D cannot be >=1");
        if (bco > 1) return fail(GD_ERR_BADARG, "unknown boundary_correction_order (expected 0 or 1)");
        if (base_F < 8 || base_F > 4096) return fail(GD_ERR_BADARG, "fine_bins_2D out of range");
        bool exchanged = false;
        if (P == 0) {
            GDB_TRY(neff_exchange(&exchanged));
            return 0;
        }
        mark("call: start", P);
        int64_t ncols = 0;
        GDB_DEV(h, ops.num_rows(h, &N, &ncols));
        if (ncols < n) return fail(GD_ERR_BADARG, "more parameters than resident columns");
        int32_t hw = 0;
        GDB_DEV(h, ops.weights_kind(h, &hw));
        unit_weights = hw == 0;
        byte_index_weights = hw == 2 && !getenv("GDHIP_NO_WSORT");
        for (int k = 0; k < P; ++k)
            if (pairs[2 * k] < 0 || pairs[2 * k] >= n || pairs[2 * k + 1] < 0 || pairs[2 * k + 1] >= n)
                return fail(GD_ERR_BADARG, "pair index out of range");
        {
            std::vector<char> seen(n, 0);
            for (int k = 0; k < 2 * P; ++k)
                if (!seen[pairs[k]]) seen[pairs[k]] = 1, used.push_back(pairs[k]);
        }
        const bool injected = ss < 0 && s.bandwidths != nullptr;
        const bool auto_bw = ss < 0 && !injected;
        bool need_neff = false;
        if (auto_bw && !s.pair_neff)
            for (int j : used) need_neff = need_neff || isnan(par[j].neff);
        void* aux = nullptr;
        const bool overlap = auto_bw && P >= 64 && twin != nullptr;
        if (overlap) {
            if (!st.aux) GDB_DEV(h, ops.create_aux(h, &st.aux));
            aux = st.aux;
        }
        std::future<int> neff_f, shear_f;
        bin_launching.store(0);
        hold_neff_for_binning = overlap && need_neff && unit_weights && !getenv("GDHIP_BATCH_NO_NEFF_HOLD");
        if (overlap && need_neff)
            neff_f = std::async(std::launch::async, [this] {
                ops.bind_thread(h);
                return neff_batch(used, true);
            });
        bmin.assign(n, NAN), bmax.assign(n, NAN);
        for (int j : used) bin_edges(par[j], &bmin[j], &bmax[j]);
        pair_scalars(s, n, corrmat, pairs, P, ps);
        fwx.resize(P), fwy.resize(P);
        for (int k = 0; k < P; ++k) {
            const int F = ps.F[k];
            if (!classes.count(F)) F_list.push_back(F);
            classes[F].push_back(k);
            fwx[k] = (bmax[ps.jx[k]] - bmin[ps.jx[k]]) / (F - 1);
            fwy[k] = (bmax[ps.jy[k]] - bmin[ps.jy[k]]) / (F - 1);
            double* m = M(k);
            for (int q = 0; q < GD_BATCH2D_META; ++q) m[q] = NAN;
            m[0] = F, m[5] = -1, m[23] = bmin[ps.jx[k]], m[24] = bmax[ps.jx[k]], m[25] = bmin[ps.jy[k]], m[26] = bmax[ps.jy[k]];
            m[27] = ps.corr[k], m[28] = (double)ps.nbin2D[k];
        }
        int64_t need = 0;
        for (int k = 0; k < P; ++k) need += (int64_t)ps.F[k] * ps.F[k];
        if (need > grids_doubles && !s.bandwidths_only) {
            if (neff_f.valid()) neff_f.get();
            return fail(GD_ERR_BADARG, "grids_pinned is too small");
        }
        std::vector<double> rngx(P), rngy(P);
        for (int k = 0; k < P; ++k) rngx[k] = bmax[ps.jx[k]] - bmin[ps.jx[k]], rngy[k] = bmax[ps.jy[k]] - bmin[ps.jy[k]];
        int rc = 0;
        if (auto_bw) {
            if (overlap) {
                const bool split_classes = F_list.size() > 1;
                bin_done.store(0);
                first_part_done.store(0);
                first_part_flag.store(nullptr), reports_enqueued = 0;
                {
                    const char* e = getenv("GDHIP_BATCH_SHEAR_DEFERRED");
                    const char* emin = getenv("GDHIP_BATCH_SHEAR_DEFERRED_MIN");
                    shear_deferred = (e ? atoi(e) != 0 : true) && unit_weights && P >= (emin ? atoi(emin) : 256);
                    if (shear_deferred && !st.aux2) {
                        int rc2 = ops.create_aux(h, &st.aux2);
                        if (!rc2 && ops.stream_priority && getenv("GDHIP_BATCH_SHEAR_LOW_PRIORITY")) rc2 = ops.stream_priority(st.aux2, -1);
                        if (rc2) {
                            if (st.aux2) ops.destroy_aux(st.aux2), st.aux2 = nullptr;
                            shear_deferred = false, (void)ops.last_error(h);
                        }
                    }
                    shear_after_binning = shear_deferred;
                }
                rc = make_plan(s, par, n, cov, ps, rngx, rngy, 0.2, plan, err);
                bins_first_rows = 0;
                bins_first_done.store(0);
                const bool will_stage = aux != nullptr && !s.want_levels && P >= s_two_min() && P > s_two_split() && !s.bandwidths_only;
                if (!rc && shear_deferred && will_stage && base_F == 256 && main_class() == 256 && !getenv("GDHIP_BATCH_ONE_BINNING")) {
                    std::vector<int>& mem = classes[256];
                    std::stable_partition(mem.begin(), mem.end(), [&](int k) { return plan.branch[k] == 2; });
                    size_t nC = 0, nA = 0;
                    for (int k : mem) nC += plan.branch[k] == 2;
                    for (int k = 0; k < P; ++k) nA += plan.branch[k] == 0;
                    if ((int)nC >= s_kopt_split_min()) {
                        const size_t part = base_part_size(nC + nA, 256), first = std::min(nC, first_part_size(part));
                        if (nC + nA > part && first < mem.size()) bins_first_rows = (int)first;
                    }
                }
                bin_joined = false, bin_rc = 0;
                bin_future = std::async(std::launch::async, [this, split_classes] {
                                 ops.bind_thread(twin);
                                 const int e = binning(twin, split_classes ? 1 : 0);
                                 bins_first_done.store(1);
                                 bin_done.store(1);
                                 return e;
                             }).share();
                if (!rc) shear_hist_state.store(0);
                if (!rc)
                    shear_f = std::async(std::launch::async, [this, aux, split_classes] {
                        void* sctx = shear_deferred ? st.aux2 : aux;
                        ops.bind_thread(sctx);
                        if (shear_after_binning) {
// ... 183 lines not shown
```

getdist_amd/csrc/ctx.hpp:

```cpp
#pragma once
#include <hip/hip_runtime.h>
#include <stdint.h>
#include <stdio.h>
#include <string.h>

#include <map>
#include <memory>
#include <mutex>
#include <set>
#include <string>
#include <atomic>
#include <vector>

#include "../../include/gdhip.h"

struct FftPlanCache;

struct BucketCols {
    std::mutex mu;
    unsigned short* buf = nullptr;
    int64_t n = 0, ld = 0;
    bool tried = false;
    std::vector<double> mn, scale;
    std::vector<int> nb;
    ~BucketCols() {
        if (buf) (void)hipFree(buf);
    }
};

#define GD_EXTRA_COLS 4

struct gd_ctx {
    int device = 0;
    hipStream_t stream = nullptr;
    hipStream_t copy_stream = nullptr;
    hipEvent_t copy_ev = nullptr;
    bool main_high = false;
    hipEvent_t ev0 = nullptr, ev1 = nullptr;
    int cu_count = 256;
    std::string err;
    double* cols = nullptr;
    double* w = nullptr;
    bool w_integral = false;
    unsigned char* w8 = nullptr;
    unsigned char* w8_main = nullptr;
    double* like_w = nullptr;
    double* w_main = nullptr;
    bool w_main_integral = false;
    double w_sum = 0, w_main_sum = 0;
    int w_sel = 0;
    bool borrowed = false;
    long long* wcum = nullptr;
    std::shared_ptr<BucketCols> bq;
    int64_t N = 0, n = 0, ld = 0;
    void* scratch = nullptr;
    int64_t scratch_bytes = 0;
    void* scratch2 = nullptr;
    int64_t scratch2_bytes = 0;
    void* gather_index = nullptr;
    int64_t gather_index_bytes = 0;
    FftPlanCache* fft = nullptr;
    std::map<int, double*> dctmat;
    std::map<int, void*> fft_tw;
    struct StageSlot {
        void* host = nullptr;
        size_t cap = 0;
        hipEvent_t ev = nullptr;
        bool used = false;
        bool own = false;
    };
    static constexpr size_t kStageBytes = 64u << 10;
    void* stage_block = nullptr;
    static constexpr int kCopyMarks = 16;
    hipEvent_t copy_marks[kCopyMarks] = {};
    int copy_mark_next = 0;
    static constexpr int kStageSlots = 32;
    StageSlot stage[kStageSlots];
    int stage_next = 0;
    struct Fetch {
        void* dst;
        size_t off, bytes;
    };
    static constexpr size_t kFetchBytes = 4u << 20, kFetchMax = 1u << 20;
    void* fetch_block = nullptr;
    size_t fetch_off = 0;
    std::vector<Fetch> fetch_pending;
    static constexpr int kKoptEvents = 32;
    hipEvent_t kopt_evs[kKoptEvents] = {};
    int kopt_ev_next = 0;
    void* comm = nullptr;
    int comm_world = 0, comm_rank = 0;
    void* comm_buf = nullptr;
    size_t comm_buf_bytes = 0;
    std::atomic<int> comm_abandon_gen{0};
    int comm_completed = 0;
    void* batch_state = nullptr;
    void (*batch_state_release)(gd_ctx*, bool destroy) = nullptr;
};

int gd_stage_h2d(gd_ctx* ctx, void* d_dst, const void* src, size_t bytes);
int gd_h2d(gd_ctx* ctx, void* d_dst, const void* src, size_t bytes);

int gd_fft_r2c_2d(gd_ctx* ctx, int n0, int n1, int batch, const double* d_in, double2* d_out);
int gd_fft_c2r_2d(gd_ctx* ctx, int n0, int n1, int batch, double2* d_in, double* d_out);
void gd_fft_cache_destroy(gd_ctx* ctx);

int gd_fetch(gd_ctx* ctx, void* host_dst, const void* d_src, size_t bytes);
int gd_fetch_pinned(gd_ctx* ctx, void* pinned_dst, const void* d_src, size_t bytes);
int gd_stream_sync(gd_ctx* ctx);

int gd_fail(gd_ctx* ctx, int code, const char* fmt, ...);
void gd_comm_release(gd_ctx* ctx);
bool gd_ctx_alive(gd_ctx* ctx);
int gd_stream_priority(gd_ctx* ctx, int level);
void* gd_scratch(gd_ctx* ctx, int64_t bytes);
void* gd_scratch2(gd_ctx* ctx, int64_t bytes);

#define GD_HIP(call)                                                                                 \
    do {                                                                                             \
        hipError_t e__ = (call);                                                                     \
        if (e__ != hipSuccess)                                                                       \
            return gd_fail(ctx, e__ == hipErrorOutOfMemory ? GD_ERR_NOMEM : GD_ERR_HIP, "%s: %s (%s:%d)", #call, \
                           hipGetErrorString(e__), __FILE__, __LINE__);                              \
    } while (0)

#define GD_KERNEL_CHECK() GD_HIP(hipGetLastError())

#define GD_TRY(call)              \
    do {                          \
        const int rc__ = (call);  \
        if (rc__) return rc__;    \
    } while (0)

#define GD_REQUIRE(cond, msg)                                   \
    do {                                                        \
        if (!(cond)) return gd_fail(ctx, GD_ERR_BADARG, "%s", msg); \
    } while (0)

#define WAVE 64

typedef double gd_f64x2 __attribute__((ext_vector_type(2)));
typedef unsigned int gd_u32x4 __attribute__((ext_vector_type(4)));
__device__ __forceinline__ double2 gload_d2(const double* p) {
    const gd_f64x2 v = *(const __attribute__((address_space(1))) gd_f64x2*)p;
    return make_double2(v.x, v.y);
}
__device__ __forceinline__ uint4 gload_u4(const void* p) {
    const gd_u32x4 v = *(const __attribute__((address_space(1))) gd_u32x4*)p;
    return make_uint4(v.x, v.y, v.z, v.w);
}

__device__ __forceinline__ double wave_sum(double v) {
#pragma unroll
    for (int o = 32; o > 0; o >>= 1) v += __shfl_down(v, o, WAVE);
    return v;
}
__device__ __forceinline__ double wave_min(double v) {
#pragma unroll
    for (int o = 32; o > 0; o >>= 1) v = fmin(v, __shfl_down(v, o, WAVE));
    return v;
}
__device__ __forceinline__ double wave_max(double v) {
#pragma unroll
    for (int o = 32; o > 0; o >>= 1) v = fmax(v, __shfl_down(v, o, WAVE));
    return v;
}

__device__ __forceinline__ double block_sum(double v, double* red) {
    v = wave_sum(v);
    const int lane = threadIdx.x & 63, wv = threadIdx.x >> 6, nw = (blockDim.x + 63) >> 6;
    __syncthreads();
    if (lane == 0) red[wv] = v;
    __syncthreads();
    double r = 0;
    if (threadIdx.x == 0)
        for (int i = 0; i < nw; ++i) r += red[i];
    return r;
}
__device__ __forceinline__ double block_min(double v, double* red) {
    v = wave_min(v);
    const int lane = threadIdx.x & 63, wv = threadIdx.x >> 6, nw = (blockDim.x + 63) >> 6;
    __syncthreads();
    if (lane == 0) red[wv] = v;
    __syncthreads();
    double r = red[0];
    if (threadIdx.x == 0)
        for (int i = 1; i < nw; ++i) r = fmin(r, red[i]);
    return r;
}
__device__ __forceinline__ double block_max(double v, double* red) {
    v = wave_max(v);
    const int lane = threadIdx.x & 63, wv = threadIdx.x >> 6, nw = (blockDim.x + 63) >> 6;
    __syncthreads();
    if (lane == 0) red[wv] = v;
    __syncthreads();
    double r = red[0];
    if (threadIdx.x == 0)
        for (int i = 1; i < nw; ++i) r = fmax(r, red[i]);
    return r;
}
```

getdist_amd/csrc/kopt2d.hip:

```cpp
#include "ctx.hpp"
#include "ldsfft.hpp"
#include "solvers.hpp"

#ifndef KT
#define KT 512
#endif
#define MAXF 6
#ifdef KOPT_PROFILE
__device__ long long g_prof[8];
__device__ long long g_wave[8];
#define PROF_T0 long long prof_t0 = clock64()
#define PROF_ADD(slot)                                                        \
    do {                                                                      \
        const long long prof_t1 = clock64();                                  \
        if (threadIdx.x == 0 && blockIdx.x == 0) g_prof[slot] += prof_t1 - prof_t0; \
        prof_t0 = prof_t1;                                                    \
    } while (0)
#else
#define PROF_T0
#define PROF_ADD(slot)
#endif
#ifndef KOPT_U
#define KOPT_U 1
#endif
#define KOPT_STRIDE 12
#define PI 3.141592653589793238462643383279502884
#define PISQ (PI * PI)

typedef double gd_f64x4 __attribute__((ext_vector_type(4)));
template <int EPI>
__global__ void __launch_bounds__(256) k_gemm_nt(const double* __restrict__ A, int64_t strideA,
                                                 const double* __restrict__ Bm, int64_t strideB, int F,
                                                 double* __restrict__ Cm, int64_t strideC,
                                                 const double* __restrict__ sums) {
    constexpr int KC = 32;
    __shared__ double As[KC][65];
    __shared__ double Bs[KC][65];
    const int b = blockIdx.z;
    const double* Ab = A + (int64_t)b * strideA;
    const double* Bb = Bm + (int64_t)b * strideB;
    const int i0 = blockIdx.y * 64, j0 = blockIdx.x * 64;
    const int lane = threadIdx.x & 63, wave = threadIdx.x >> 6;
    const int wi = (wave >> 1) * 32, wj = (wave & 1) * 32;
    const int l15 = lane & 15, lk = lane >> 4;
    gd_f64x4 acc[2][2];
#pragma unroll
    for (int u = 0; u < 2; ++u)
#pragma unroll
        for (int v = 0; v < 2; ++v) acc[u][v] = (gd_f64x4){0.0, 0.0, 0.0, 0.0};
    constexpr int NQ = 64 * KC / 256;
    double ra[NQ], rb[NQ];
    auto fetch = [&](int p0) {
#pragma unroll
        for (int q = 0; q < NQ; ++q) {
            const int e = threadIdx.x + 256 * q;
            const int pp = e & (KC - 1), ii = e / KC;
            const int p = p0 + pp;
            ra[q] = (i0 + ii < F && p < F) ? Ab[(int64_t)(i0 + ii) * F + p] : 0.0;
            rb[q] = (j0 + ii < F && p < F) ? Bb[(int64_t)(j0 + ii) * F + p] : 0.0;
        }
    };
    fetch(0);
    for (int p0 = 0; p0 < F; p0 += KC) {
        __syncthreads();
#pragma unroll
        for (int q = 0; q < NQ; ++q) {
            const int e = threadIdx.x + 256 * q;
            As[e & (KC - 1)][e / KC] = ra[q];
            Bs[e & (KC - 1)][e / KC] = rb[q];
        }
        __syncthreads();
        if (p0 + KC < F) fetch(p0 + KC);
#pragma unroll
        for (int kk = 0; kk < KC / 4; ++kk) {
            const int k = kk * 4 + lk;
            const double a0 = As[k][wi + l15], a1 = As[k][wi + 16 + l15];
            const double b0 = Bs[k][wj + l15], b1 = Bs[k][wj + 16 + l15];
            acc[0][0] = __builtin_amdgcn_mfma_f64_16x16x4f64(a0, b0, acc[0][0], 0, 0, 0);
            acc[0][1] = __builtin_amdgcn_mfma_f64_16x16x4f64(a0, b1, acc[0][1], 0, 0, 0);
            acc[1][0] = __builtin_amdgcn_mfma_f64_16x16x4f64(a1, b0, acc[1][0], 0, 0, 0);
            acc[1][1] = __builtin_amdgcn_mfma_f64_16x16x4f64(a1, b1, acc[1][1], 0, 0, 0);
        }
    }
    double* Cb = Cm + (int64_t)b * strideC;
    const double inv = (EPI == 1) ? sums[b] : 1.0;
#pragma unroll
    for (int u = 0; u < 2; ++u)
#pragma unroll
        for (int v = 0; v < 2; ++v)
#pragma unroll
            for (int r = 0; r < 4; ++r) {
                const int i = i0 + wi + u * 16 + lk + 4 * r, j = j0 + wj + v * 16 + l15;
                if (i < F && j < F) {
                    if (EPI == 0) {
                        Cb[(int64_t)i * F + j] = acc[u][v][r];
                    } else {
                        const double val = acc[u][v][r] / inv;
                        Cb[(int64_t)j * F + i] = val * val;
                    }
                }
            }
}


template <int EPI, bool BIG>
__global__ void __launch_bounds__(512) k_dct_pass(const double* __restrict__ src, int F, FftDev plH, const double2* __restrict__ twg,
                                                  const double2* __restrict__ cg, const double* __restrict__ sums,
                                                  double* __restrict__ dst) {
    extern __shared__ double2 dsh[];
    const int H = F >> 1, b = blockIdx.y, RPB = blockDim.x / FT;
    double2* tw = dsh;
    double2* ck = dsh + F;
    const int g = threadIdx.x / FT, t = threadIdx.x % FT;
    double2* buf = dsh + 2 * F + (size_t)g * F;
    double* stage = (double*)(buf + H);
    const int row = blockIdx.x * RPB + g;
    const bool active = row < F;
    {
        const double* x = src + (int64_t)b * F * F + (int64_t)min(row, F - 1) * F;
        for (int i0 = t; i0 < F; i0 += 8 * FT) {
            double xv[8];
#pragma unroll
            for (int q = 0; q < 8; ++q) xv[q] = x[min(i0 + q * FT, F - 1)];
            __builtin_amdgcn_sched_barrier(0);
#pragma unroll
            for (int q = 0; q < 8; ++q) stage[min(i0 + q * FT, F - 1)] = xv[q];
        }
        for (int i0 = threadIdx.x; i0 < F; i0 += 2 * blockDim.x) {
            const int i1 = min(i0 + (int)blockDim.x, F - 1);
            const double2 a0 = twg[i0], a1 = twg[i1], c0 = cg[i0], c1 = cg[i1];
            __builtin_amdgcn_sched_barrier(0);
            tw[i0] = a0, tw[i1] = a1, ck[i0] = c0, ck[i1] = c1;
        }
    }
    __syncthreads();
    if (active) {
        auto v = [&](int m) { return m < H ? stage[2 * m] : stage[2 * (F - 1 - m) + 1]; };
        for (int n = t; n < H; n += FT) buf[n] = make_double2(v(2 * n), v(2 * n + 1));
    }
    group_sync();
    fft_full<BIG, false>(buf, tw, 2, plH, t);
    if (active) {
        const double inv = EPI == 1 ? sums[b] : 1.0;
        auto put = [&](int k, double y) {
            if (EPI == 1) {
                const double val = y / inv;
                stage[k] = val * val;
            } else {
                stage[k] = y;
            }
        };
        for (int k = t; 2 * k <= H; k += FT) {
            if (k == 0) {
                const double2 z = buf[0];
                put(0, 2.0 * (z.x + z.y));
                const double vh = z.x - z.y;
                put(H, 2.0 * (ck[H].x * vh));
                continue;
            }
            const double2 zk = buf[k], zm = buf[H - k];
            const double ax = zk.x + zm.x, ay = zk.y - zm.y, bx = zk.x - zm.x, by = zk.y + zm.y;
            {
                const double2 e = tw[k];
                const double u = fma(e.x, bx, -(e.y * by)), w = fma(e.x, by, e.y * bx);
                const double vx = 0.5 * (ax + w), vy = 0.5 * (ay - u);
                const double2 c1 = ck[k], c2 = ck[F - k];
                put(k, 2.0 * fma(c1.x, vx, -(c1.y * vy)));
                put(F - k, 2.0 * fma(c2.x, vx, c2.y * vy));
            }
            if (2 * k < H) {
                const double2 f = tw[H - k];
                const double u2 = -fma(f.x, bx, f.y * by), w2 = fma(f.x, by, -(f.y * bx));
                const double vx = 0.5 * (ax + w2), vy = 0.5 * (-ay - u2);
                const double2 c1 = ck[H - k], c2 = ck[H + k];
                put(H - k, 2.0 * fma(c1.x, vx, -(c1.y * vy)));
                put(H + k, 2.0 * fma(c2.x, vx, c2.y * vy));
            }
        }
    }
    __syncthreads();
    double* out = dst + (int64_t)b * F * F + (int64_t)blockIdx.x * RPB;
    const int nrows = min(RPB, F - blockIdx.x * RPB);
    for (int e = threadIdx.x; e < F * RPB; e += blockDim.x) {
        const int k = e / RPB, r = e - k * RPB;
        if (r < nrows) {
            const double* st = (const double*)(dsh + 2 * F + (size_t)r * F + H);
            out[(int64_t)k * F + r] = st[k];
        }
    }
}

__global__ void k_dct_matrix(int F, double* __restrict__ D) {
    const int e = blockIdx.x * blockDim.x + threadIdx.x;
    if (e >= F * F) return;
    const int k = e / F, n = e % F;
    const long long m = ((long long)k * (2 * n + 1)) % (4LL * F);
    const int q = (int)(m / F);
    const int r = (int)(m - (long long)q * F);
    const double c = cospi((double)r / (2.0 * F)), s = sinpi((double)r / (2.0 * F));
    double v = (q == 0) ? c : (q == 1) ? -s : (q == 2) ? -c : s;
    D[e] = 2.0 * v;
}

__global__ void k_hist_sums(const double* __restrict__ hist, int FF, double* __restrict__ sums) {
    __shared__ double red[16];
    const double* h = hist + (int64_t)blockIdx.x * FF;
    double s = 0;
    for (int i = threadIdx.x; i < FF; i += blockDim.x) s += h[i];
    s = block_sum(s, red);
    if (threadIdx.x == 0) sums[blockIdx.x] = s;
}

__global__ void k_gather_norm(const double* __restrict__ hist, const int* __restrict__ which, const double* __restrict__ sums,
                              int FF, double* __restrict__ out) {
    const int b = which[blockIdx.y];
    const double s = sums[b];
    for (int i = blockIdx.x * blockDim.x + threadIdx.x; i < FF; i += gridDim.x * blockDim.x)
        out[(int64_t)blockIdx.y * FF + i] = hist[(int64_t)b * FF + i] / s;
}

__global__ void k_power_full(const double2* __restrict__ Z, int F, double* __restrict__ out) {
    const int Fh = F / 2 + 1;
    const double2* Zb = Z + (int64_t)blockIdx.y * F * Fh;
    double* ob = out + (int64_t)blockIdx.y * F * F;
    for (int e = blockIdx.x * blockDim.x + threadIdx.x; e < F * F; e += gridDim.x * blockDim.x) {
        const int i = e / F, j = e % F;
        double2 z;
        if (j < Fh)
            z = Zb[(int64_t)i * Fh + j];
        else
            z = Zb[(int64_t)((F - i) % F) * Fh + (F - j)];
        ob[e] = z.x * z.x + z.y * z.y;
    }
}

struct KoptLds {
    double* wx;
    double* wy;
    double* res;
    double* red;
    double* times;
    double* scale;
    double* tile;
    int tile_doubles;
};

__device__ void bilinear_forms_reg(const double* __restrict__ M, int F, int m, KoptLds L, int kmax);

__device__ void bilinear_forms(const double* __restrict__ M, int F, int m, KoptLds L, int kmax) {
    if (L.tile == nullptr) {
        bilinear_forms_reg(M, F, m, L, kmax);
        return;
    }
    const int lane = threadIdx.x & 63, wave = threadIdx.x >> 6;
    const int nseg = (kmax + 127) >> 7;
    const int rows_fit = L.tile_doubles / (nseg * 128);
    const int jx = threadIdx.x & 127, g = threadIdx.x >> 7;
    double val[MAXF];
#pragma unroll
    for (int q = 0; q < MAXF; ++q) val[q] = 0;
    PROF_T0;
    for (int r0 = 0; r0 < kmax; r0 += rows_fit) {
        const int nr = min(rows_fit, kmax - r0);
        for (int idx = wave; idx < nr * nseg; idx += KT / 64) {
            const int row = idx / nseg, seg = idx - row * nseg;
            __builtin_amdgcn_global_load_lds(
                (const __attribute__((address_space(1))) void*)(M + (int64_t)(r0 + row) * F + seg * 128 + lane * 2),
                (__attribute__((address_space(3))) void*)(L.tile + idx * 128), 16, 0, 0);
        }
        __syncthreads();
        PROF_ADD(1);
        for (int j0 = 0; j0 < nseg * 128; j0 += 256) {
            const int j = j0 + 2 * jx;
            if (j < kmax) {
                double ax[MAXF], ay[MAXF];
#pragma unroll
                for (int q = 0; q < MAXF; ++q) ax[q] = ay[q] = 0;
                const double* col = L.tile + (j >> 7) * 128 + (j & 127);
                for (int r = 2 * g; r < nr; r += 2 * (KT / 128)) {
                    const double2 a0 = *reinterpret_cast<const double2*>(col + r * nseg * 128);
                    const bool two = r + 1 < nr;
                    const double2 a1 = two ? *reinterpret_cast<const double2*>(col + (r + 1) * nseg * 128)
                                           : make_double2(0.0, 0.0);
#pragma unroll
                    for (int q = 0; q < MAXF; ++q)
                        if (q < m) {
                            const double2 wyq = *reinterpret_cast<const double2*>(L.wy + q * F + r0 + r);
                            ax[q] = fma(wyq.x, a0.x, ax[q]);
                            ay[q] = fma(wyq.x, a0.y, ay[q]);
                            const double wy1 = two ? wyq.y : 0.0;
                            ax[q] = fma(wy1, a1.x, ax[q]);
                            ay[q] = fma(wy1, a1.y, ay[q]);
                        }
                }
#pragma unroll
                for (int q = 0; q < MAXF; ++q)
                    if (q < m) {
                        val[q] = fma(ax[q], L.wx[q * F + j], val[q]);
                        if (j + 1 < kmax) val[q] = fma(ay[q], L.wx[q * F + j + 1], val[q]);
                    }
            }
        }
        __syncthreads();
        PROF_ADD(2);
    }
    const int wv = wave;
#pragma unroll
    for (int q = 0; q < MAXF; ++q)
        if (q < m) {
            const double r = wave_sum(val[q]);
            if (lane == 0) L.wx[q * 16 + wv] = r;
        }
    __syncthreads();
    if ((int)threadIdx.x < m) {
        double r = 0;
        for (int i = 0; i < KT / 64; ++i) r += L.wx[threadIdx.x * 16 + i];
        L.res[threadIdx.x] = r;
    }
    __syncthreads();
    PROF_ADD(3);
}

__device__ void bilinear_forms_reg(const double* __restrict__ M, int F, int m, KoptLds L, int kmax) {
    constexpr int U = KOPT_U;
    const int jx = threadIdx.x & 127, g = threadIdx.x >> 7;
    const int rows_per = (kmax + KT / 128 - 1) / (KT / 128);
    const int r_lo = g * rows_per, r_hi = min(kmax, r_lo + rows_per);
    double val[MAXF];
#pragma unroll
    for (int q = 0; q < MAXF; ++q) val[q] = 0;
    for (int j0 = 0; j0 < kmax; j0 += 256) {
        const int j = j0 + 2 * jx;
        if (j < kmax) {
            double ax[MAXF], ay[MAXF];
#pragma unroll
            for (int q = 0; q < MAXF; ++q) ax[q] = ay[q] = 0;
            for (int i = r_lo; i < r_hi; i += U) {
                double2 a[U];
#pragma unroll
                for (int u = 0; u < U; ++u)
                    a[u] = (i + u < r_hi) ? *reinterpret_cast<const double2*>(M + (int64_t)(i + u) * F + j)
                                          : make_double2(0.0, 0.0);
#pragma unroll
                for (int u = 0; u < U; ++u) {
                    const int iu = min(i + u, r_hi - 1);
#pragma unroll
                    for (int q = 0; q < MAXF; ++q)
                        if (q < m) {
                            const double wyq = L.wy[q * F + iu];
                            ax[q] = fma(wyq, a[u].x, ax[q]);
                            ay[q] = fma(wyq, a[u].y, ay[q]);
                        }
                }
            }
#pragma unroll
            for (int q = 0; q < MAXF; ++q)
                if (q < m) {
                    val[q] = fma(ax[q], L.wx[q * F + j], val[q]);
                    if (j + 1 < kmax) val[q] = fma(ay[q], L.wx[q * F + j + 1], val[q]);
                }
        }
    }
    __syncthreads();
    const int lane = threadIdx.x & 63, wv = threadIdx.x >> 6;
#pragma unroll
    for (int q = 0; q < MAXF; ++q)
        if (q < m) {
            const double r = wave_sum(val[q]);
            if (lane == 0) L.wx[q * 16 + wv] = r;
        }
    __syncthreads();
// ... 574 lines not shown
            wxs[idx] = v;
            wys[(mf - 1 - q) * KR_F + k] = v;
        } else {
            (isy ? wys : wxs)[idx] = v;
        }
    }
}

template <bool ODD>
__global__ void __launch_bounds__(KR_T) k_kopt2d_res(const double* __restrict__ M_all, const KoptPair* __restrict__ pairs,
                                                     double* __restrict__ out) {
    extern __shared__ double lds[];
    KresView V;
    V.wxs = lds;
    V.wys = lds + MAXF * KR_F;
    V.mt = V.wys + MAXF * KR_F;
    V.logI = V.mt + 8 * KR_LDS * KR_F;
    V.sh = reinterpret_cast<KresShared*>(V.logI + KR_F);
    KresShared* S = V.sh;
    const int b = blockIdx.x, w = threadIdx.x >> 6, l = threadIdx.x & 63;
    double* o = out + (int64_t)b * KOPT_STRIDE;
    if (ODD && !(pairs[b].do_corr && o[7] == (double)GD_OK)) return;
    double m[KR_REG][4];
    RPROF_T0;
    kres_load(M_all + (int64_t)(ODD ? pairs[b].pw_index : b) * KR_F * KR_F, m, V.mt, w, l);
    if (!ODD) {
        if (threadIdx.x < 6) S->scale[threadIdx.x] = pow(PI, (double)(2 * threadIdx.x));
        if (threadIdx.x >= 64 && threadIdx.x < 64 + 5 * MAXF) {
            const int Ls = (threadIdx.x - 64) / MAXF, a = (threadIdx.x - 64) % MAXF;
            if (a <= Ls) {
                const double cst = (1.0 + pow(0.5, (double)(Ls + 1))) / 3.0;
                S->ceven[Ls][a] = -2.0 * cst * k_even(a) * k_even(Ls - a);
            }
        }
        if (threadIdx.x >= 256) V.logI[threadIdx.x - 256] = log((double)(threadIdx.x - 256) * (double)(threadIdx.x - 256));
    } else {
        if (threadIdx.x >= 8 && threadIdx.x < 14) S->scale[threadIdx.x - 2] = pow(2.0 * PI, (double)(2 * (threadIdx.x - 8)));
        if (threadIdx.x >= 128 && threadIdx.x < 138) S->kodd[threadIdx.x - 128] = k_odd(threadIdx.x - 128);
        if (threadIdx.x >= 192 && threadIdx.x < 195) {
            const int Ls = 4 + 2 * (threadIdx.x - 192);
            S->codd[threadIdx.x - 192] = 8.0 * (1.0 - pow(2.0, (double)(-Ls - 1))) / 3.0;
        }
    }
    if (threadIdx.x == 0) {
        const KoptPair P = pairs[b];
        S->N = P.N, S->fallback_t = P.fallback_t, S->do_corr = P.do_corr;
        S->xpre = 0.0, S->xcur = 0.1, S->xblk = 0.0, S->fblk = 0.0, S->spre = 0.0, S->scur = 0.0, S->t_star = 0.0;
        S->fpre = 0.0, S->fcur = 0.0;
        S->status = GD_OK, S->done = 0, S->it = -2;
        S->x = 0.0;
        if (!ODD) {
            S->stage = KR_STAGE_BRENT, S->Ls = 5, S->Lmin = 2, S->t = 0.0;
        } else {
            S->stage = KR_STAGE_ODD, S->Ls = 10, S->Lmin = 4, S->t = o[0];
            S->p00 = o[4];
        }
        for (int q = 0; q < MAXF; ++q) S->times[q] = S->t;
    }
    for (int e = threadIdx.x; e < 6 * MAXF; e += KR_T) (&S->lev[0][0])[e] = 0.0;
#ifdef KOPT_PROFILE
    if (threadIdx.x < 8) S->prof[threadIdx.x] = 0, S->wave_cycles[threadIdx.x] = 0;
#endif
    __syncthreads();
    RPROF_ADD(1);
#pragma unroll 1
    for (;;) {
        const int stage = S->stage, Ls = S->Ls;
        if (stage == KR_STAGE_EXIT) break;
        const int mf = ODD ? Ls / 2 : Ls + 1;
        kres_weights<ODD>(V.wxs, V.wys, V.logI, S->times, Ls, mf, Ls == (ODD ? 10 : 5), threadIdx.x);
        RPROF_ADD(0);
        __syncthreads();
        RPROF_ADD(5);
        kres_forms(m, V, mf, w, l);
        __syncthreads();
        RPROF_ADD(3);
        if (threadIdx.x < MAXF) kres_tail<ODD>(S, Ls, threadIdx.x);
        RPROF_ADD(7);
        __syncthreads();
        RPROF_ADD(4);
    }
#ifdef KOPT_PROFILE
    if (threadIdx.x < 8 && blockIdx.x == 0 && !ODD) g_prof[threadIdx.x] += S->prof[threadIdx.x], g_wave[threadIdx.x] += S->wave_cycles[threadIdx.x];
#endif
    if (threadIdx.x == 0) {
        if (!ODD) {
            const bool ok = S->status == GD_OK;
            const bool dc = ok && S->do_corr;
            o[0] = ok ? S->t_star : NAN;
            o[1] = ok ? S->lev[2][0] : NAN, o[2] = ok ? S->lev[2][2] : NAN, o[3] = ok ? S->lev[2][1] : NAN;
            o[4] = dc ? S->lev[0][0] : NAN;
            o[5] = NAN, o[6] = NAN;
            o[7] = (double)S->status;
        } else {
            o[5] = S->odd[0][0];
            o[6] = S->odd[0][1];
        }
    }
}

__global__ void __launch_bounds__(64) k_get_h(double* __restrict__ kopt, const double* __restrict__ neff,
                                              const double* __restrict__ corr, const int* __restrict__ do_corr, int B) {
    const int b = blockIdx.x;
    if (b >= B || threadIdx.x >= 4) return;
    double* o = kopt + (int64_t)b * KOPT_STRIDE;
    const bool ok = o[7] == (double)GD_OK;
    double psi[6];
    for (int q = 0; q < 6; ++q) psi[q] = o[1 + q];
    if (!ok) {
        if (threadIdx.x == 0) o[8] = o[9] = o[10] = NAN, o[11] = (double)GD_ERR_SOLVER;
        return;
    }
    const gdsolve::GetHResult r = gdsolve::get_h(psi, neff[b], corr[b], do_corr[b] != 0);
    if (threadIdx.x == 0) {
        o[8] = r.hx, o[9] = r.hy, o[10] = r.corr;
        o[11] = r.status ? (double)GD_ERR_BADARG : (double)GD_OK;
    }
}

extern "C" {

int gd_get_h(gd_ctx* ctx, int32_t B, const double* psi, const double* neff, const double* corr, const int32_t* do_corr,
             double* out) {
    GD_REQUIRE(ctx && psi && neff && corr && do_corr && out && B > 0, "bad argument");
    int64_t off = 0;
    auto take = [&](int64_t bytes) {
        int64_t o = off;
        off += (bytes + 255) / 256 * 256;
        return o;
    };
    const int64_t o_k = take((int64_t)B * KOPT_STRIDE * 8), o_n = take((int64_t)B * 8), o_c = take((int64_t)B * 8),
                  o_d = take((int64_t)B * 4);
    char* base = (char*)gd_scratch(ctx, off);
    if (!base) return GD_ERR_NOMEM;
    std::vector<double> hk((size_t)B * KOPT_STRIDE, 0.0);
    for (int b = 0; b < B; ++b) {
        for (int q = 0; q < 6; ++q) hk[(size_t)b * KOPT_STRIDE + 1 + q] = psi[(size_t)b * 6 + q];
        hk[(size_t)b * KOPT_STRIDE + 7] = (double)GD_OK;
    }
    GD_TRY(gd_h2d(ctx, base + o_k, hk.data(), hk.size() * 8));
    GD_TRY(gd_h2d(ctx, base + o_n, neff, (size_t)B * 8));
    GD_TRY(gd_h2d(ctx, base + o_c, corr, (size_t)B * 8));
    GD_TRY(gd_h2d(ctx, base + o_d, do_corr, (size_t)B * 4));
    k_get_h<<<B, 64, 0, ctx->stream>>>((double*)(base + o_k), (const double*)(base + o_n), (const double*)(base + o_c),
                                      (const int*)(base + o_d), B);
    GD_KERNEL_CHECK();
    GD_TRY(gd_fetch(ctx, hk.data(), base + o_k, hk.size() * 8));
    GD_TRY(gd_stream_sync(ctx));
    for (int b = 0; b < B; ++b)
        for (int q = 0; q < 4; ++q) out[(size_t)b * 4 + q] = hk[(size_t)b * KOPT_STRIDE + 8 + q];
    return GD_OK;
}

static int kopt_stage_a(gd_ctx* ctx, int32_t B, int32_t F, const void* d_hist_v, const double* neff, const int32_t* do_corr,
                        const double* fallback_t, double* d_rows) {
    GD_REQUIRE(ctx && d_hist_v && neff && do_corr && fallback_t && d_rows && B > 0, "bad argument");
    GD_REQUIRE(F >= 16 && F <= 1024, "KernelOptimizer2D grid size out of range (16..1024)");
    const double* d_hist = (const double*)d_hist_v;
    const int64_t FF = (int64_t)F * F;
    FftDev plH;
    const double2 *d_tw = nullptr, *d_ck = nullptr;
    bool dct_fft = F % 2 == 0 && F / 2 <= 512 && F >= 64 && getenv("GDHIP_KOPT_DCT_GEMM") == nullptr &&
                   lds_fft_plan(ctx, F / 2, &plH, nullptr);
    if (dct_fft) {
        FftDev plF;
        dct_fft = lds_fft_plan(ctx, F, &plF, &d_tw);
    }
    if (dct_fft) {
        auto it = ctx->fft_tw.find(-F);
        if (it == ctx->fft_tw.end()) {
            std::vector<double2> hck((size_t)F);
            for (int k = 0; k < F; ++k) {
                const long double a = -3.141592653589793238462643383279502884L * (long double)k / (2.0L * (long double)F);
                hck[k] = make_double2((double)cosl(a), (double)sinl(a));
            }
            void* d = nullptr;
            GD_HIP(hipMalloc(&d, (size_t)F * 16));
            if (hipMemcpy(d, hck.data(), (size_t)F * 16, hipMemcpyHostToDevice) != hipSuccess) {
                (void)hipFree(d);
                return gd_fail(ctx, GD_ERR_HIP, "upload of the DCT post-twiddles failed");
            }
            it = ctx->fft_tw.emplace(-F, d).first;
        }
        d_ck = (const double2*)it->second;
    }
    double* D = nullptr;
    if (!dct_fft) {
        auto it = ctx->dctmat.find(F);
        if (it == ctx->dctmat.end()) {
            GD_HIP(hipMalloc((void**)&D, (size_t)FF * 8));
            k_dct_matrix<<<(unsigned)((FF + 255) / 256), 256, 0, ctx->stream>>>(F, D);
            GD_KERNEL_CHECK();
            ctx->dctmat[F] = D;
        } else {
            D = it->second;
        }
    }
    std::vector<KoptPair> hp((size_t)B);
    std::vector<int> which;
    for (int b = 0; b < B; ++b) {
        hp[b].N = neff[b];
        hp[b].fallback_t = fallback_t[b];
        hp[b].do_corr = do_corr[b] ? 1 : 0;
        hp[b].pw_index = -1;
        if (do_corr[b]) {
            hp[b].pw_index = (int)which.size();
            which.push_back(b);
        }
    }
    const int nc = (int)which.size();
    const int Fh = F / 2 + 1;
    int64_t off = 0;
    auto take = [&](int64_t bytes) {
        int64_t o = off;
        off += (bytes + 255) / 256 * 256;
        return o;
    };
    const int64_t o_pairs = take((int64_t)B * sizeof(KoptPair)), o_which = take((int64_t)(nc + 1) * 4);
    const int64_t table_bytes = off;
    const int64_t o_sums = take((int64_t)B * 8), o_E = take((int64_t)B * FF * 8),
                  o_SQ = take((int64_t)B * FF * 8), o_Z = take((int64_t)nc * F * Fh * 16), o_PW = take((int64_t)nc * FF * 8);
    char* base = (char*)gd_scratch(ctx, off);
    if (!base) return GD_ERR_NOMEM;
    double* d_sums = (double*)(base + o_sums);
    KoptPair* d_pairs = (KoptPair*)(base + o_pairs);
    double* d_out = d_rows;
    int* d_which = (int*)(base + o_which);
    double* d_E = (double*)(base + o_E);
    double* d_SQ = (double*)(base + o_SQ);
    double2* d_Z = (double2*)(base + o_Z);
    double* d_PW = (double*)(base + o_PW);
    {
        std::vector<char> tab((size_t)table_bytes, 0);
        memcpy(tab.data() + o_pairs, hp.data(), (size_t)B * sizeof(KoptPair));
        if (nc) memcpy(tab.data() + o_which, which.data(), (size_t)nc * 4);
        GD_TRY(gd_stage_h2d(ctx, base, tab.data(), (size_t)table_bytes));
    }
    k_hist_sums<<<B, 1024, 0, ctx->stream>>>(d_hist, (int)FF, d_sums);
    GD_KERNEL_CHECK();
    if (dct_fft) {
        const int RPB = F <= 256 ? 16 : (F <= 512 ? 8 : 4);
        const size_t lds = ((size_t)2 * F + (size_t)RPB * F) * 16;
        const dim3 grid((F + RPB - 1) / RPB, B);
        const bool big = F / 2 > 320;
        auto k0 = big ? k_dct_pass<0, true> : k_dct_pass<0, false>;
        auto k1 = big ? k_dct_pass<1, true> : k_dct_pass<1, false>;
        GD_HIP(hipFuncSetAttribute((const void*)k0, hipFuncAttributeMaxDynamicSharedMemorySize, (int)lds));
        GD_HIP(hipFuncSetAttribute((const void*)k1, hipFuncAttributeMaxDynamicSharedMemorySize, (int)lds));
        k0<<<grid, RPB * FT, lds, ctx->stream>>>(d_hist, F, plH, d_tw, d_ck, nullptr, d_E);
        GD_KERNEL_CHECK();
        k1<<<grid, RPB * FT, lds, ctx->stream>>>(d_E, F, plH, d_tw, d_ck, d_sums, d_SQ);
        GD_KERNEL_CHECK();
    } else {
        const dim3 ggrid((F + 63) / 64, (F + 63) / 64, B);
        k_gemm_nt<0><<<ggrid, 256, 0, ctx->stream>>>(D, 0, d_hist, FF, F, d_E, FF, nullptr);
        GD_KERNEL_CHECK();
        k_gemm_nt<1><<<ggrid, 256, 0, ctx->stream>>>(d_E, FF, D, 0, F, d_SQ, FF, d_sums);
        GD_KERNEL_CHECK();
    }
    if (nc > 0) {
        k_gather_norm<<<dim3(64, nc), 256, 0, ctx->stream>>>(d_hist, d_which, d_sums, (int)FF, d_E);
        GD_KERNEL_CHECK();
        int rc = gd_fft_r2c_2d(ctx, F, F, nc, d_E, d_Z);
        if (rc) return rc;
        k_power_full<<<dim3(64, nc), 256, 0, ctx->stream>>>(d_Z, F, d_PW);
        GD_KERNEL_CHECK();
    }
    const size_t lds_base = ((size_t)2 * MAXF * F + 8 + 16 + 8 + 16) * 8;
    size_t tile_bytes = 0;
    if (F % 128 == 0 && getenv("GDHIP_KOPT_NO_LDS_TILE") == nullptr) {
        const size_t room = (size_t)160 * 1024 - 1024 - lds_base;
        size_t cap = (size_t)128 * 1024;
        if (const char* e = getenv("GDHIP_KOPT_TILE_KB")) cap = (size_t)atoi(e) * 1024;
        tile_bytes = room < cap ? room : cap;
        tile_bytes = tile_bytes / ((size_t)F * 8) * ((size_t)F * 8);
    }
    const size_t lds = lds_base + tile_bytes;
    if (F == KR_F && getenv("GDHIP_KOPT_STREAMED") == nullptr) {
        const size_t lds_res = ((size_t)2 * MAXF * KR_F + (size_t)8 * KR_LDS * KR_F + KR_F) * 8 + sizeof(KresShared);
        GD_HIP(hipFuncSetAttribute((const void*)k_kopt2d_res<false>, hipFuncAttributeMaxDynamicSharedMemorySize, (int)lds_res));
        k_kopt2d_res<false><<<B, KR_T, lds_res, ctx->stream>>>(d_SQ, d_pairs, d_out);
        if (nc > 0) {
            GD_KERNEL_CHECK();
            GD_HIP(hipFuncSetAttribute((const void*)k_kopt2d_res<true>, hipFuncAttributeMaxDynamicSharedMemorySize, (int)lds_res));
            k_kopt2d_res<true><<<B, KR_T, lds_res, ctx->stream>>>(d_PW, d_pairs, d_out);
        }
    } else {
        GD_HIP(hipFuncSetAttribute((const void*)k_kopt2d, hipFuncAttributeMaxDynamicSharedMemorySize, (int)lds));
        k_kopt2d<<<B, KT, lds, ctx->stream>>>(d_SQ, d_PW, d_pairs, F, (int)(tile_bytes / 8), d_out);
    }
    GD_KERNEL_CHECK();
#ifdef KOPT_PROFILE
    {
        long long hp[8];
        GD_TRY(gd_stream_sync(ctx));
        GD_HIP(hipMemcpyFromSymbol(hp, HIP_SYMBOL(g_prof), sizeof(hp)));
        fprintf(stderr, "kopt block 0 cycles: weights %lld  tile-load %lld  tile-fma %lld  reduce %lld  "
                        "entry-barrier %lld  times/pow %lld | levels (streamed) or barrier after the weights (resident) %lld  kmax sum %lld\n",
                hp[0], hp[1], hp[2], hp[3], hp[4], hp[7], hp[5], hp[6]);
        long long hw[8];
        GD_HIP(hipMemcpyFromSymbol(hw, HIP_SYMBOL(g_wave), sizeof(hw)));
        fprintf(stderr, "  forms per wave: %lld %lld %lld %lld %lld %lld %lld %lld\n", hw[0], hw[1], hw[2], hw[3], hw[4], hw[5], hw[6], hw[7]);
        memset(hp, 0, sizeof(hp));
        GD_HIP(hipMemcpyToSymbol(HIP_SYMBOL(g_prof), hp, sizeof(hp)));
        GD_HIP(hipMemcpyToSymbol(HIP_SYMBOL(g_wave), hp, sizeof(hp)));
    }
#endif
    return GD_OK;
}

#define KOPT_BLOCK_DOUBLES 15
static int kopt_stage_b(gd_ctx* ctx, hipEvent_t after, int32_t B, double* d_rows, double* out) {
    GD_REQUIRE(ctx && d_rows && out && B > 0, "bad argument");
    if (after) GD_HIP(hipStreamWaitEvent(ctx->stream, after, 0));
    const double* d_neff = d_rows + (int64_t)B * KOPT_STRIDE;
    const double* d_corr = d_neff + B;
    const int* d_dc = (const int*)(d_corr + B);
    k_get_h<<<B, 64, 0, ctx->stream>>>(d_rows, d_neff, d_corr, d_dc, B);
    GD_KERNEL_CHECK();
    GD_TRY(gd_fetch(ctx, out, d_rows, (size_t)B * KOPT_STRIDE * 8));
    GD_TRY(gd_stream_sync(ctx));
    return GD_OK;
}

static int kopt_upload_get_h_inputs(gd_ctx* ctx, int32_t B, double* d_rows, const double* neff, const double* corr,
                                    const int32_t* do_corr) {
    std::vector<double> tab((size_t)3 * B, 0.0);
    memcpy(tab.data(), neff, (size_t)B * 8);
    memcpy(tab.data() + B, corr, (size_t)B * 8);
    memcpy(tab.data() + 2 * (size_t)B, do_corr, (size_t)B * 4);
    return gd_h2d(ctx, d_rows + (int64_t)B * KOPT_STRIDE, tab.data(), tab.size() * 8);
}

int gd_kopt2d(gd_ctx* ctx, int32_t B, int32_t F, const void* d_hist_v, const double* neff, const int32_t* do_corr,
              const double* fallback_t, const double* corr, double* out) {
    GD_REQUIRE(ctx && d_hist_v && neff && do_corr && fallback_t && corr && out && B > 0, "bad argument");
    double* d_rows = (double*)gd_scratch2(ctx, (int64_t)B * KOPT_BLOCK_DOUBLES * 8);
    if (!d_rows) return GD_ERR_NOMEM;
    GD_TRY(kopt_upload_get_h_inputs(ctx, B, d_rows, neff, corr, do_corr));
    GD_TRY(kopt_stage_a(ctx, B, F, d_hist_v, neff, do_corr, fallback_t, d_rows));
    return kopt_stage_b(ctx, nullptr, B, d_rows, out);
}

int gd_kopt2d_enqueue(gd_ctx* ctx, int32_t B, int32_t F, const void* d_hist, const double* neff, const int32_t* do_corr,
                      const double* fallback_t, const double* corr, void* d_rows, int32_t* ticket_out) {
    GD_REQUIRE(ctx && ticket_out && d_rows && neff && corr && do_corr && B > 0, "bad argument");
    GD_TRY(kopt_upload_get_h_inputs(ctx, B, (double*)d_rows, neff, corr, do_corr));
    GD_TRY(kopt_stage_a(ctx, B, F, d_hist, neff, do_corr, fallback_t, (double*)d_rows));
    const int slot = ctx->kopt_ev_next;
    ctx->kopt_ev_next = (slot + 1) % gd_ctx::kKoptEvents;
    if (!ctx->kopt_evs[slot]) GD_HIP(hipEventCreateWithFlags(&ctx->kopt_evs[slot], hipEventDisableTiming));
    GD_HIP(hipEventRecord(ctx->kopt_evs[slot], ctx->stream));
    *ticket_out = slot;
    return GD_OK;
}

int gd_kopt2d_finish(gd_ctx* ctx, gd_ctx* stage_a_ctx, int32_t ticket, int32_t B, void* d_rows, double* out) {
    GD_REQUIRE(ctx && stage_a_ctx && ticket >= 0 && ticket < gd_ctx::kKoptEvents && stage_a_ctx->kopt_evs[ticket], "bad ticket");
    GD_HIP(hipSetDevice(ctx->device));
    return kopt_stage_b(ctx, ctx == stage_a_ctx ? nullptr : stage_a_ctx->kopt_evs[ticket], B, (double*)d_rows, out);
}

}
```

include/gdhip.h:

```cpp
#ifndef GDHIP_H
#define GDHIP_H

#include <stdint.h>

#ifdef __cplusplus
extern "C" {
#endif

typedef struct gd_ctx gd_ctx;

typedef enum gd_status {
    GD_OK = 0,
    GD_ERR_BADARG = -1,
    GD_ERR_NOMEM = -2,
    GD_ERR_HIP = -3,
    GD_ERR_EMPTY = -4,
    GD_ERR_SOLVER = -5,
    GD_ERR_FFT = -6,
    GD_ERR_NODEVICE = -7,
    GD_ERR_TIMEOUT = -8
} gd_status;

int gd_device_count(void);
int gd_create(int device, gd_ctx** out);
void gd_destroy(gd_ctx* ctx);
const char* gd_last_error(gd_ctx* ctx);
const char* gd_version(void);
int gd_device_info(gd_ctx* ctx, int64_t* info6);
int gd_sync(gd_ctx* ctx);
int gd_dev_alloc(gd_ctx* ctx, int64_t bytes, void** d_out);
int gd_dev_free(gd_ctx* ctx, void* d_ptr);
int gd_memcpy_h2d(gd_ctx* ctx, void* d_dst, const void* src, int64_t bytes);
int gd_memcpy_d2h(gd_ctx* ctx, void* dst, const void* d_src, int64_t bytes);
int gd_memcpy_d2h_async(gd_ctx* ctx, void* dst, const void* d_src, int64_t bytes);
int gd_copy_sync(gd_ctx* ctx);
int gd_copy_mark(gd_ctx* ctx, int32_t* token_out);
int gd_copy_wait(gd_ctx* ctx, int32_t token);
int gd_memcpy_d2d(gd_ctx* ctx, void* d_dst, const void* d_src, int64_t bytes);
int gd_memset(gd_ctx* ctx, void* d_dst, int value, int64_t bytes);
int gd_gather_items(gd_ctx* ctx, void* d_dst, const void* d_src, const int32_t* index, int32_t count, int64_t item_bytes);
int gd_host_alloc(gd_ctx* ctx, int64_t bytes, void** out);
int gd_host_free(gd_ctx* ctx, void* ptr);
int gd_timer_start(gd_ctx* ctx);
int gd_timer_stop_ms(gd_ctx* ctx, double* ms_out);

int gd_upload(gd_ctx* ctx, const double* X, int64_t N, int64_t n, int64_t row_stride, int64_t col_stride,
              const double* weights);
int gd_num_rows(gd_ctx* ctx, int64_t* N, int64_t* n);
int gd_column_ptr(gd_ctx* ctx, int64_t j, void** d_out);

int gd_weight_stats(gd_ctx* ctx, int64_t row_lo, int64_t row_hi, double thresh, double* out4);
int gd_col_stats(gd_ctx* ctx, int64_t row_lo, int64_t row_hi, double* out);
int gd_cov(gd_ctx* ctx, const int32_t* cols, int32_t m, int64_t row_lo, int64_t row_hi, double* means_out,
           double* cov_out, double* norm_out, double* minmax_out);

int gd_quantiles(gd_ctx* ctx, const int32_t* cols, int32_t ncols, int64_t row_lo, int64_t row_hi,
                 const double* targets, int32_t k, double* out);

int gd_quantiles_mm(gd_ctx* ctx, const int32_t* cols, int32_t ncols, int64_t row_lo, int64_t row_hi,
                    const double* targets, int32_t k, const double* minmax, double* out);

int gd_quantiles_mm_probe(gd_ctx* ctx, const int32_t* cols, int32_t ncols, int64_t row_lo, int64_t row_hi,
                          const double* targets, int32_t k, const double* minmax, double* out, const double* probe_means,
                          double* probe_out, int32_t* probe_done);

int gd_autocov_lags(gd_ctx* ctx, int32_t col, double mean, int64_t k0, int32_t nlags, double* out);
int gd_kde_lag_sums(gd_ctx* ctx, int32_t col, double inv4s2, const int64_t* lags, int32_t nlags, double* out);
int gd_kde_lag_sums_2d(gd_ctx* ctx, int32_t coli, int32_t colj, const double* kinv3, const int64_t* lags, int32_t nlags,
                       double* out);
int gd_autocov_lags_batch(gd_ctx* ctx, const int32_t* cols, int32_t ncols, const double* means, int64_t k0,
                          int32_t nlags, double* out);
int gd_kde_lag_sums_batch(gd_ctx* ctx, const int32_t* cols, int32_t ncols, const double* inv4s2, const int64_t* lags,
                          int32_t nlags, double* out);
int gd_autocov_lags_range_batch(gd_ctx* ctx, const int32_t* cols, int32_t ncols, const double* means, int64_t row_lo,
                                int64_t row_hi, int64_t k0, int32_t nlags, double* out);

int gd_hist1d(gd_ctx* ctx, const int32_t* cols, int32_t ncols, const double* binmin, const double* width,
              int32_t F, double* out);
int gd_hist1d_dev(gd_ctx* ctx, const int32_t* cols, int32_t ncols, const double* binmin, const double* width,
                  int32_t F, void* d_out);
int gd_bin_indices(gd_ctx* ctx, int32_t col, double binmin, double width, int32_t round_half, int32_t F,
                   int32_t* idx_out, int64_t* n_out_of_range);
int gd_prebin(gd_ctx* ctx, int32_t col, double binmin, double width, int32_t F, void* d_idx_u16);
int gd_prebin8_batch(gd_ctx* ctx, const int32_t* cols, int32_t ncols, const double* binmin, const double* width, int32_t F,
                     void* const* d_idx_out, int64_t* bad_out);
int gd_hist2d_prebinned8(gd_ctx* ctx, int32_t B, const void* const* d_idx_x, const void* const* d_idx_y, void* d_hist);
int gd_prebin8_hist2d(gd_ctx* ctx, const int32_t* cols, int32_t ncols, const double* binmin, const double* width,
                      void* const* d_idx_out, int64_t* bad_out, int32_t B, const void* const* d_idx_x,
                      const void* const* d_idx_y, void* d_hist);

int gd_prebin_batch(gd_ctx* ctx, const int32_t* cols, int32_t ncols, const double* binmin, const double* width, int32_t F,
                    void* const* d_idx_u16);
int gd_hist2d(gd_ctx* ctx, int32_t B, const int32_t* colx, const int32_t* coly, const double* binminx,
              const double* widthx, const double* binminy, const double* widthy, int32_t F, void* d_hist);
int gd_hist2d_prebinned(gd_ctx* ctx, int32_t B, const void* const* d_idx_x, const void* const* d_idx_y, int32_t F,
                        void* d_hist);
int gd_minmax_affine(gd_ctx* ctx, int32_t B, const int32_t* coli, const int32_t* colj, const double* a,
                     const double* b, double* out);
int gd_hist2d_sheared(gd_ctx* ctx, int32_t B, const int32_t* coli, const int32_t* colj, const double* r0,
                      const double* r1, const double* xmin, const double* dx, const double* ymin, const double* dy,
                      int32_t F, void* d_hist);

int gd_isj1d(gd_ctx* ctx, int32_t B, int32_t F, const double* hist, const double* neff, double* hfrac_out,
             int32_t* status_out);
int gd_isj1d_dev(gd_ctx* ctx, int32_t B, int32_t F, const void* d_hist, const double* neff, double* hfrac_out,
                 int32_t* status_out);

int gd_dct1d(gd_ctx* ctx, int32_t B, int32_t F, const double* hist, double* a_out);
int gd_density1d(gd_ctx* ctx, int32_t B, int32_t F, const double* hist, const double* smooth, const int32_t* winw,
                 const int32_t* flags, int32_t bco, int32_t mbc, double* P_out, int32_t* status_out);
int gd_density1d_dev(gd_ctx* ctx, int32_t B, int32_t F, const void* d_hist, const double* smooth, const int32_t* winw,
                     const int32_t* flags, int32_t bco, int32_t mbc, double* P_out, int32_t* status_out);

int gd_kopt2d(gd_ctx* ctx, int32_t B, int32_t F, const void* d_hist, const double* neff, const int32_t* do_corr,
              const double* fallback_t, const double* corr, double* out);
#define GD_KOPT_BLOCK_DOUBLES 15
int gd_kopt2d_enqueue(gd_ctx* ctx, int32_t B, int32_t F, const void* d_hist, const double* neff, const int32_t* do_corr,
                      const double* fallback_t, const double* corr, void* d_rows, int32_t* ticket_out);
int gd_kopt2d_finish(gd_ctx* ctx, gd_ctx* stage_a_ctx, int32_t ticket, int32_t B, void* d_rows, double* out);
int gd_get_h(gd_ctx* ctx, int32_t B, const double* psi, const double* neff, const double* corr, const int32_t* do_corr,
             double* out);

int gd_density2d(gd_ctx* ctx, int32_t B, int32_t F, const void* d_hist, const double* rx, const double* ry,
                 const double* corr, const int32_t* winw, const int32_t* flags, int32_t bco, int32_t mbc,
                 void* d_P_out, int32_t* status_out);
int gd_density2d_enqueue(gd_ctx* ctx, int32_t B, int32_t F, const void* d_hist, const double* rx, const double* ry,
                         const double* corr, const int32_t* winw, const int32_t* flags, int32_t bco, int32_t mbc,
                         void* d_P_out, int32_t* status_pinned);

int gd_density2d_enqueue_indexed(gd_ctx* ctx, int32_t B, int32_t F, const void* d_hist, const int32_t* hist_index,
                                 const double* rx, const double* ry, const double* corr, const int32_t* winw,
                                 const int32_t* flags, int32_t bco, int32_t mbc, void* d_P_out, int32_t* status_pinned);

int gd_attach_samples(gd_ctx* ctx, gd_ctx* owner);
int gd_bind_thread(gd_ctx* ctx);

int gd_contour_levels(gd_ctx* ctx, int32_t B, int32_t F, const void* d_P, const double* contours, int32_t nc, double* out,
                      int32_t* status_out);

int gd_limits1d(gd_ctx* ctx, int32_t B, int32_t F, const double* P, const double* x0, const double* spacing,
                const double* contours, int32_t nc, int32_t factor, double* out, int32_t* status_out);

int gd_set_extra_column(gd_ctx* ctx, int32_t slot, const double* x);
int gd_aux_weights(gd_ctx* ctx, const double* w);
int gd_col_minmax(gd_ctx* ctx, const int32_t* cols, int32_t ncols, int64_t lo, int64_t hi, int32_t cond_col,
                  double cond_below, double* out);

int gd_weights_integral(gd_ctx* ctx, int32_t* out);
int gd_thin_rows(gd_ctx* ctx, int64_t lo, int64_t hi, int64_t factor, int32_t unique_mode, void* d_rows, int64_t capacity,
                 int64_t* count_out);
int gd_binary_transitions(gd_ctx* ctx, const int32_t* cols, int32_t ncols, const void* d_rows, int64_t K,
                          const double* thresholds, int32_t nthr, int64_t* counts_out);
int gd_thinned_lag_sums(gd_ctx* ctx, const int32_t* cols, int32_t ncols, const double* means, const void* d_rows, int64_t K,
                        int32_t maxoff, double* out);

int gd_like_weights(gd_ctx* ctx, const double* loglikes, int32_t mode, double mean_loglike, double* sum_out);
int gd_select_weights(gd_ctx* ctx, int32_t which);
int gd_likes1d(gd_ctx* ctx, int32_t B, int32_t F, const double* hist, const double* likehist, const double* P,
               const double* smooth, const int32_t* winw, const int32_t* flags, int32_t shade_mean_loglikes,
               double* likes_out, int32_t* status_out);
int gd_likes2d(gd_ctx* ctx, int32_t B, int32_t F, const void* d_hist, const void* d_likehist, const double* rx,
               const double* ry, const double* corr, const int32_t* winw, const int32_t* flags, int32_t mbc,
               void* d_likes_out, int32_t* status_out);

int gd_density2d_masked(gd_ctx* ctx, int32_t F, const void* d_hist, double rx, double ry, double corr, int32_t winw,
                        int32_t flags, int32_t bco, int32_t mbc, const double* mask_bc, const double* mask_mbc,
                        const unsigned char* zero_mask, void* d_P_out, int32_t* status_out);

#define GD_HISTND_MAXD 25
#define GD_HISTND_MAX_BINS (1 << 25)
#define GD_HISTND_H 1
#define GD_HISTND_LIKES 2
#define GD_HISTND_LMIN 4
int gd_histnd_batch(gd_ctx* ctx, int32_t B, const int32_t* dims, const int32_t* cols, const double* binmin,
                    const double* width, int32_t nb, int32_t flags, int32_t loglike_col, double* H_out, double* HL_out,
                    double* Lmin_out);

#define GD_PCA_MAX_PROJ 448
int gd_pca_corr(gd_ctx* ctx, const int32_t* cols, int32_t n, const int32_t* maps, double* mean_out, double* sd_out,
                double* corr_out);
int gd_pca_project(gd_ctx* ctx, const int32_t* cols, int32_t np, const int32_t* maps, const double* mean, const double* sd,
                   const double* U, int32_t doexp, int32_t n_all, const double* all_means, const double* all_sd,
                   double* newmean_out, double* newsd_out, double* pcpc_out, double* pcpar_out);

int gd_mixture_nll(gd_ctx* ctx, const int32_t* cols, int32_t d, int32_t K, const double* means, const double* whiten,
                   const double* logcoef, int64_t row_lo, int64_t row_hi, double* out);

int gd_circ_convolve(gd_ctx* ctx, int32_t n0, int32_t n1, const double* a, const double* b, double* out);
int gd_convolve1d_direct(gd_ctx* ctx, const double* x, int64_t nx, const double* y, int64_t ny, double* out_full);
int gd_autoconvolve(gd_ctx* ctx, int32_t col, double mean, int32_t use_weights, const double* x_host, int64_t nx, int64_t s,
                    int64_t n, int32_t normalize, double* out);

int gd_like_stats(gd_ctx* ctx, int32_t col, double* out8);


#define GD_BATCH2D_META 32
#define GD_BATCH2D_NEED_NEFF (-20)

typedef struct gd_param2d {
    double range_min, range_max;
    double param_min, param_max;
    double sigma_range, err;
    double mean, var;
    double neff;
    int32_t has_limits_bot, has_limits_top, periodic;
    int32_t owned;
} gd_param2d;

typedef struct gd_batch2d_settings {
    int32_t fine_bins_2D, boundary_correction_order, mult_bias_correction_order, num_bins_2D;
    double smooth_scale_2D, max_corr_2D;
    double norm, sum_w2;
    int32_t uncorrelated_sampler;
    int32_t raise_on_bandwidth_errors;
    int32_t want_levels, ncontours;
    const double* contours;
    int32_t two_streams_min;
    int32_t two_streams_split;
    int32_t kopt_split_min;
    double kopt_first_fraction;
    int32_t first_batch, max_batch;
    double max_batch_bytes;
    int32_t comm_exchange;
    int32_t bandwidths_only;
    const double* pair_neff;
    const double* bandwidths;
    int32_t results_in_flight;
} gd_batch2d_settings;

typedef int (*gd_neff_exchange_fn)(void* user, double* neff_n, int32_t n);

int gd_batch2d_grid_sizes(const gd_batch2d_settings* settings, int32_t n, const double* corr, const int32_t* pairs,
                          int32_t P, int32_t* F_out);
int gd_density2d_batch(gd_ctx* ctx, gd_ctx* twin, const gd_batch2d_settings* settings, gd_param2d* params, int32_t n,
                       const double* corr, const double* cov, const double* lag_probe, const int32_t* pairs, int32_t P,
                       gd_neff_exchange_fn exchange, void* exchange_user, void* grids_pinned, int64_t grids_doubles,
                       int32_t* status_pinned, double* meta, double* levels, int32_t* level_status, int32_t* tokens_out2);
#define GD_BATCH1D_META 9

typedef struct gd_density1d_settings {
    int32_t fine_bins, num_bins, boundary_correction_order, mult_bias_correction_order;
    double smooth_scale_1D;
    double norm, sum_w2;
    int32_t uncorrelated_sampler;
    int32_t raise_on_bandwidth_errors;
} gd_density1d_settings;

int gd_density1d_batch(gd_ctx* ctx, const gd_density1d_settings* settings, gd_param2d* params, int32_t n, const int32_t* cols,
                       int32_t B, double* P_out, double* hist_out, double* meta);

int gd_batch2d_finish(gd_ctx* ctx);
int gd_batch2d_invalidate(gd_ctx* ctx);
int gd_batch2d_exchanges(gd_ctx* ctx, int64_t* count_out);


int gd_comm_rccl_path(char* buf, int32_t len, int32_t* preloaded_out);
int gd_upload_shard(gd_ctx* ctx, const double* X_cols, int64_t N, int64_t n, int64_t col_first, int64_t col_count,
                    int64_t col_stride, const double* weights);
int gd_comm_share_columns(gd_ctx* ctx, const int64_t* first_by_rank );
int gd_comm_unique_id(void* id128_out);
int gd_comm_init(gd_ctx* ctx, int32_t world, int32_t rank, const void* id128);
int gd_comm_info(gd_ctx* ctx, int32_t* world_out, int32_t* rank_out);
int gd_comm_abandon(gd_ctx* ctx);
int gd_comm_destroy(gd_ctx* ctx);
int gd_comm_allgather(gd_ctx* ctx, const double* send, int64_t count, double* recv);
int gd_comm_allreduce_sum(gd_ctx* ctx, double* inout, int64_t count);
int gd_comm_allgather_dev(gd_ctx* ctx, const void* d_send, int64_t count, void* d_recv);
int gd_comm_allreduce_sum_dev(gd_ctx* ctx, const void* d_send, int64_t count, void* d_recv);

#ifdef __cplusplus
}
#endif
// ... 2 lines not shown
```

Baseline: 50160.

## Read kernel-optimiser histograms in place via row pointers and skip known sums

The 2D kernel-width optimiser now reads histograms where they already sit, either as a contiguous run or through a per-row device pointer table. This replaces gathering them into a pooled batch buffer with device copies. For unit-weight binned histograms it also passes the known total (sample count) so the per-histogram sum reduction is skipped for those rows. The cost is extra pointer tables in scratch, indirect loads in the DCT/GEMM kernels, and extra bookkeeping of which histogram rows are complete.

Measured after the change: 50270, median of 2. Within noise of the previous version (+0.2%).

```diff
diff --git a/getdist_amd/_lib.py b/getdist_amd/_lib.py
--- a/getdist_amd/_lib.py
+++ b/getdist_amd/_lib.py
@@ -96,6 +96,9 @@
     "gd_kopt2d": (C.c_int, [_p, _i32, _i32, _p, _pd, _pi32, _pd, _pd, _pd]),
     "gd_kopt2d_enqueue": (C.c_int, [_p, _i32, _i32, _p, _pd, _pi32, _pd, _pd, _p, _pi32]),
     "gd_kopt2d_finish": (C.c_int, [_p, _p, _i32, _i32, _p, _pd]),
+    "gd_kopt2d_src": (C.c_int, [_p, _i32, _i32, _p, C.POINTER(C.c_void_p), _pd, _pd, _pi32, _pd, _pd, _pd]),
+    "gd_kopt2d_enqueue_src": (C.c_int, [_p, _i32, _i32, _p, C.POINTER(C.c_void_p), _pd, _pd, _pi32, _pd, _pd, _p, _pi32]),
+    "gd_kopt2d_sums": (C.c_int, [_p, _i32, _pd]),
     "gd_get_h": (C.c_int, [_p, _i32, _pd, _pd, _pd, _pi32, _pd]),
     "gd_density2d": (C.c_int, [_p, _i32, _i32, _p, _pd, _pd, _pd, _pi32, _pi32, _i32, _i32, _p, _pi32]),
     "gd_copy_mark": (C.c_int, [_p, _pi32]),
@@ -884,6 +887,17 @@
                                        _ip(do_corr), _dp(fallback_t), _dp(corr), _dp(out)))
         return out
 
+    def kopt2d_src(self, d_hist, B, F, neff, do_corr, fallback_t, corr, row_ptrs=None, known_sum=None):
+        neff, do_corr, fallback_t, corr = _f64arr(neff), _i32arr(do_corr), _f64arr(fallback_t), _f64arr(corr)
+        out, sums = np.zeros((B, 12)), np.zeros(B)
+        rows = None if row_ptrs is None else (C.c_void_p * B)(*[int(p) for p in row_ptrs])
+        known = None if known_sum is None else _f64arr(known_sum)
+        base = None if d_hist is None else (d_hist.ptr if isinstance(d_hist, DevBuf) else d_hist)
+        self._check(self.lib.gd_kopt2d_src(self.h, B, F, base, rows, None if known is None else _dp(known), _dp(neff),
+                                           _ip(do_corr), _dp(fallback_t), _dp(corr), _dp(out)))
+        self._check(self.lib.gd_kopt2d_sums(self.h, B, _dp(sums)))
+        return out, sums
+
     def get_h(self, psi, neff, corr, do_corr):
         psi, neff, corr, do_corr = _f64arr(psi).reshape(-1, 6), _f64arr(neff), _f64arr(corr), _i32arr(do_corr)
         out = np.zeros((len(psi), 4))
diff --git a/getdist_amd/csrc/batch2d.hip b/getdist_amd/csrc/batch2d.hip
--- a/getdist_amd/csrc/batch2d.hip
+++ b/getdist_amd/csrc/batch2d.hip
@@ -96,6 +96,17 @@
      [](void* ctx, int level) { return gd_stream_priority(C(ctx), level); },
     [](void* h, const int32_t* cols, int32_t ncols, const double* binmin, const double* width, int32_t F, void* const* d_idx) {
         return gd_prebin_batch(C(h), cols, ncols, binmin, width, F, d_idx);
+    },
+};
+
+const gdb::KoptSrcOps kKoptSrc = {
+    [](void* h, int32_t B, int32_t F, const void* d_hist, const void* const* row_ptrs, const double* known_sum, const double* neff,
+       const int32_t* do_corr, const double* fallback_t, const double* corr, double* out) {
+        return gd_kopt2d_src(C(h), B, F, d_hist, row_ptrs, known_sum, neff, do_corr, fallback_t, corr, out);
+    },
+    [](void* h, int32_t B, int32_t F, const void* d_hist, const void* const* row_ptrs, const double* known_sum, const double* neff,
+       const int32_t* do_corr, const double* fallback_t, const double* corr, void* d_rows, int32_t* ticket) {
+        return gd_kopt2d_enqueue_src(C(h), B, F, d_hist, row_ptrs, known_sum, neff, do_corr, fallback_t, corr, d_rows, ticket);
     },
 };
 
@@ -164,6 +175,7 @@
     try {
         gdb::Call call(state_of(ctx), kOps, ctx, twin, *settings, params, n, corr, cov, lag_probe, pairs, P, exchange, exchange_user,
                        (double*)grids_pinned, grids_doubles, status_pinned, meta, levels, level_status);
+        call.kopt_src = &kKoptSrc;
         rc = call.run(tokens_out2);
         if (rc) ctx->err = call.err;
     } catch (const std::exception& e) {
diff --git a/getdist_amd/csrc/batch2d.hpp b/getdist_amd/csrc/batch2d.hpp
--- a/getdist_amd/csrc/batch2d.hpp
+++ b/getdist_amd/csrc/batch2d.hpp
@@ -70,6 +70,14 @@
                         void* const* d_idx);
 };
 
+struct KoptSrcOps {
+    int (*kopt2d_src)(void* h, int32_t B, int32_t F, const void* d_hist, const void* const* row_ptrs, const double* known_sum,
+                      const double* neff, const int32_t* do_corr, const double* fallback_t, const double* corr, double* out);
+    int (*kopt2d_enqueue_src)(void* h, int32_t B, int32_t F, const void* d_hist, const void* const* row_ptrs,
+                              const double* known_sum, const double* neff, const int32_t* do_corr, const double* fallback_t,
+                              const double* corr, void* d_rows, int32_t* ticket);
+};
+
 static inline double py_pow(double x, double y) {
     volatile double e = y;
     return pow(x, e);
@@ -427,6 +435,7 @@
           pairs(pairs_), P(P_), exchange(ex_), exchange_user(ex_user_), grids(grids_), grids_doubles(grids_doubles_),
           status_pinned(status_), meta(meta_), levels(levels_), level_status(level_status_), pool{st_, ops_, h_} {}
 
+    const KoptSrcOps* kopt_src = nullptr;
     int64_t N = 0;
     bool unit_weights = true;
     Pool pool;
@@ -450,6 +459,8 @@
     std::vector<int32_t> flags, group;
     std::vector<void*> call_blocks;
     std::vector<void*> bin_stale;
+    void* u8_buf = nullptr;
+    int u8_rows_ok = 0;
     std::mutex enq_mu;
     std::atomic<int> bin_launching{0};
     bool hold_neff_for_binning = false;
@@ -809,16 +820,22 @@
                     {
                         std::lock_guard<std::mutex> g(enq_mu);
                         hists[F] = d;
+                        if (unit_weights) u8_buf = d, u8_rows_ok = B1;
                     }
                     published = true;
                     bins_first_done.store(1);
                     e = ops.hist2d_prebinned8(ctx, B - B1, ix.data() + B1, iy.data() + B1, (char*)d + (int64_t)B1 * 65536 * 8);
                     mark("binning: the other rows done", B - B1);
-                    if (e == 0) continue;
+                    if (e == 0) {
+                        std::lock_guard<std::mutex> g(enq_mu);
+                        if (unit_weights) u8_rows_ok = B;
+                        continue;
+                    }
                 }
                 if (e == 0) {
                     std::lock_guard<std::mutex> g(enq_mu);
                     hists[F] = d;
+                    if (unit_weights) u8_buf = d, u8_rows_ok = B;
                     continue;
                 }
                 if (published) {
@@ -1087,6 +1104,8 @@
         bool whole = false;
         void* d_batch = nullptr;
         bool own = false;
+        std::vector<const void*> src;
+        std::vector<double> known;
         void* d_rows = nullptr;
         int32_t ticket = -1;
         std::vector<double> ne, fb, ci;
@@ -1116,7 +1135,17 @@
         const int B = (int)L.ks.size(), F = L.F;
         const int64_t item = (int64_t)F * F * 8;
         L.d_batch = L.d_hist, L.own = false;
-        if (!L.whole) {
+        L.src.clear(), L.known.clear();
+        const bool in_place = kopt_src != nullptr && getenv("GDHIP_KOPT_GATHER") == nullptr;
+        bool run = L.na == 0 && !L.pos.empty();
+        for (size_t q = 1; q < L.pos.size() && run; ++q) run = L.pos[q] == L.pos[q - 1] + 1;
+        if (!L.whole && in_place && run) {
+            L.d_batch = (char*)L.d_hist + (int64_t)L.pos[0] * item;
+        } else if (!L.whole && in_place) {
+            L.d_batch = nullptr;
+            for (int a = 0; a < L.na; ++a) L.src.push_back((const char*)shear.d_rot + (int64_t)a * item);
+            for (int q : L.pos) L.src.push_back((const char*)L.d_hist + (int64_t)q * item);
+        } else if (!L.whole) {
             int rc = 0;
             L.d_batch = pool.take((int64_t)B * item, &rc);
             if (!L.d_batch) return dev_fail(rc, h);
@@ -1139,7 +1168,32 @@
             L.fb[row] = rowA ? -1.0 : plan.fallback_t[k];
             L.ci[row] = rowA ? 0.0 : ps.actual[k];
         }
+        if (kopt_src) {
+            L.known.assign(B, NAN);
+            std::lock_guard<std::mutex> g(enq_mu);
+            if (u8_buf && L.d_hist == u8_buf && L.F == 256)
+                for (size_t q = 0; q < L.pos.size(); ++q)
+                    if (L.pos[q] < u8_rows_ok) L.known[(size_t)L.na + q] = (double)N;
+        }
+        int nknown = 0;
+        for (double v : L.known) nknown += !isnan(v);
+        mark(L.own ? "kopt: histograms gathered" : (L.d_batch == nullptr ? "kopt: histograms in place, pointer table"
+             : (L.d_batch == L.d_hist ? "kopt: histograms in place, from the head of the block" : "kopt: histograms in place, a run of rows")),
+             B, nknown);
         return 0;
+    }
+    int launch_kopt(Launch& L, double* out) {
+        const int B = (int)L.ks.size();
+        if (kopt_src) {
+            const void* const* rows = L.src.empty() ? nullptr : L.src.data();
+            if (out)
+                return kopt_src->kopt2d_src(h, B, L.F, L.d_batch, rows, L.known.data(), L.ne.data(), L.dc.data(), L.fb.data(),
+                                            L.ci.data(), out);
+            return kopt_src->kopt2d_enqueue_src(h, B, L.F, L.d_batch, rows, L.known.data(), L.ne.data(), L.dc.data(), L.fb.data(),
+                                                L.ci.data(), L.d_rows, &L.ticket);
+        }
+        if (out) return ops.kopt2d(h, B, L.F, L.d_batch, L.ne.data(), L.dc.data(), L.fb.data(), L.ci.data(), out);
+        return ops.kopt2d_enqueue(h, B, L.F, L.d_batch, L.ne.data(), L.dc.data(), L.fb.data(), L.ci.data(), L.d_rows, &L.ticket);
     }
 
     int absorb_rows(const Launch& L, const std::vector<double>& out) {
@@ -1297,7 +1351,7 @@
                 std::vector<double> out((size_t)B * 12);
                 if (!rc) {
                     mark("kopt: launch", B, L.F);
-                    rc = ops.kopt2d(h, B, L.F, L.d_batch, L.ne.data(), L.dc.data(), L.fb.data(), L.ci.data(), out.data());
+                    rc = launch_kopt(L, out.data());
                     mark("kopt: done");
                     if (rc) dev_fail(rc, h);
                 }
@@ -1386,7 +1440,7 @@
                 }
                 if (!rc) {
                     mark("kopt: stage A enqueue", q, B);
-                    rc = ops.kopt2d_enqueue(h, B, L.F, L.d_batch, L.ne.data(), L.dc.data(), L.fb.data(), L.ci.data(), L.d_rows, &L.ticket);
+                    rc = launch_kopt(L, nullptr);
                     if (rc) dev_fail(rc, h);
                 }
                 std::lock_guard<std::mutex> g(mu);
diff --git a/getdist_amd/csrc/ctx.hpp b/getdist_amd/csrc/ctx.hpp
--- a/getdist_amd/csrc/ctx.hpp
+++ b/getdist_amd/csrc/ctx.hpp
@@ -88,6 +88,8 @@
     static constexpr int kKoptEvents = 32;
     hipEvent_t kopt_evs[kKoptEvents] = {};
     int kopt_ev_next = 0;
+    const double* kopt_sums = nullptr;
+    int kopt_sums_count = 0;
     void* comm = nullptr;
     int comm_world = 0, comm_rank = 0;
     void* comm_buf = nullptr;
diff --git a/getdist_amd/csrc/kopt2d.hip b/getdist_amd/csrc/kopt2d.hip
--- a/getdist_amd/csrc/kopt2d.hip
+++ b/getdist_amd/csrc/kopt2d.hip
@@ -32,13 +32,14 @@
 __global__ void __launch_bounds__(256) k_gemm_nt(const double* __restrict__ A, int64_t strideA,
                                                  const double* __restrict__ Bm, int64_t strideB, int F,
                                                  double* __restrict__ Cm, int64_t strideC,
-                                                 const double* __restrict__ sums) {
+                                                 const double* __restrict__ sums,
+                                                 const double* const* __restrict__ Brows = nullptr) {
     constexpr int KC = 32;
     __shared__ double As[KC][65];
     __shared__ double Bs[KC][65];
     const int b = blockIdx.z;
     const double* Ab = A + (int64_t)b * strideA;
-    const double* Bb = Bm + (int64_t)b * strideB;
+    const double* Bb = Brows ? Brows[b] : Bm + (int64_t)b * strideB;
     const int i0 = blockIdx.y * 64, j0 = blockIdx.x * 64;
     const int lane = threadIdx.x & 63, wave = threadIdx.x >> 6;
     const int wi = (wave >> 1) * 32, wj = (wave & 1) * 32;
@@ -106,7 +107,7 @@
 template <int EPI, bool BIG>
 __global__ void __launch_bounds__(512) k_dct_pass(const double* __restrict__ src, int F, FftDev plH, const double2* __restrict__ twg,
                                                   const double2* __restrict__ cg, const double* __restrict__ sums,
-                                                  double* __restrict__ dst) {
+                                                  double* __restrict__ dst, const double* const* __restrict__ rows = nullptr) {
     extern __shared__ double2 dsh[];
     const int H = F >> 1, b = blockIdx.y, RPB = blockDim.x / FT;
     double2* tw = dsh;
@@ -117,7 +118,7 @@
     const int row = blockIdx.x * RPB + g;
     const bool active = row < F;
     {
-        const double* x = src + (int64_t)b * F * F + (int64_t)min(row, F - 1) * F;
+        const double* x = (rows ? rows[b] : src + (int64_t)b * F * F) + (int64_t)min(row, F - 1) * F;
         for (int i0 = t; i0 < F; i0 += 8 * FT) {
             double xv[8];
 #pragma unroll
@@ -202,21 +203,22 @@
     D[e] = 2.0 * v;
 }
 
-__global__ void k_hist_sums(const double* __restrict__ hist, int FF, double* __restrict__ sums) {
+__global__ void k_hist_sums(const double* const* __restrict__ rows, const int* __restrict__ todo, int FF, double* __restrict__ sums) {
     __shared__ double red[16];
-    const double* h = hist + (int64_t)blockIdx.x * FF;
+    const int b = todo[blockIdx.x];
+    const double* h = rows[b];
     double s = 0;
     for (int i = threadIdx.x; i < FF; i += blockDim.x) s += h[i];
     s = block_sum(s, red);
-    if (threadIdx.x == 0) sums[blockIdx.x] = s;
-}
-
-__global__ void k_gather_norm(const double* __restrict__ hist, const int* __restrict__ which, const double* __restrict__ sums,
+    if (threadIdx.x == 0) sums[b] = s;
+}
+
+__global__ void k_gather_norm(const double* const* __restrict__ wrows, const int* __restrict__ which, const double* __restrict__ sums,
                               int FF, double* __restrict__ out) {
-    const int b = which[blockIdx.y];
-    const double s = sums[b];
+    const double* h = wrows[blockIdx.y];
+    const double s = sums[which[blockIdx.y]];
     for (int i = blockIdx.x * blockDim.x + threadIdx.x; i < FF; i += gridDim.x * blockDim.x)
-        out[(int64_t)blockIdx.y * FF + i] = hist[(int64_t)b * FF + i] / s;
+        out[(int64_t)blockIdx.y * FF + i] = h[i] / s;
 }
 
 __global__ void k_power_full(const double2* __restrict__ Z, int F, double* __restrict__ out) {
@@ -1097,12 +1099,18 @@
     return GD_OK;
 }
 
-static int kopt_stage_a(gd_ctx* ctx, int32_t B, int32_t F, const void* d_hist_v, const double* neff, const int32_t* do_corr,
-                        const double* fallback_t, double* d_rows) {
-    GD_REQUIRE(ctx && d_hist_v && neff && do_corr && fallback_t && d_rows && B > 0, "bad argument");
+static int kopt_stage_a(gd_ctx* ctx, int32_t B, int32_t F, const void* d_hist_v, const void* const* row_ptrs,
+                        const double* known_sum, const double* neff, const int32_t* do_corr, const double* fallback_t,
+                        double* d_rows) {
+    GD_REQUIRE(ctx && (d_hist_v || row_ptrs) && neff && do_corr && fallback_t && d_rows && B > 0, "bad argument");
     GD_REQUIRE(F >= 16 && F <= 1024, "KernelOptimizer2D grid size out of range (16..1024)");
-    const double* d_hist = (const double*)d_hist_v;
     const int64_t FF = (int64_t)F * F;
+    if (getenv("GDHIP_KOPT_SUM_PASS")) known_sum = nullptr;
+    std::vector<const double*> hrows((size_t)B);
+    for (int b = 0; b < B; ++b) {
+        hrows[b] = row_ptrs ? (const double*)row_ptrs[b] : (const double*)d_hist_v + (int64_t)b * FF;
+        GD_REQUIRE(hrows[b], "null histogram pointer");
+    }
     FftDev plH;
     const double2 *d_tw = nullptr, *d_ck = nullptr;
     bool dct_fft = F % 2 == 0 && F / 2 <= 512 && F >= 64 && getenv("GDHIP_KOPT_DCT_GEMM") == nullptr &&
@@ -1142,7 +1150,9 @@
         }
     }
     std::vector<KoptPair> hp((size_t)B);
-    std::vector<int> which;
+    std::vector<int> which, todo;
+    std::vector<const double*> wrows;
+    std::vector<double> hsums((size_t)B, NAN);
     for (int b = 0; b < B; ++b) {
         hp[b].N = neff[b];
         hp[b].fallback_t = fallback_t[b];
@@ -1151,9 +1161,14 @@
         if (do_corr[b]) {
             hp[b].pw_index = (int)which.size();
             which.push_back(b);
-        }
-    }
-    const int nc = (int)which.size();
+            wrows.push_back(hrows[b]);
+        }
+        if (known_sum && !isnan(known_sum[b]))
+            hsums[b] = known_sum[b];
+        else
+            todo.push_back(b);
+    }
+    const int nc = (int)which.size(), ntodo = (int)todo.size();
     const int Fh = F / 2 + 1;
     int64_t off = 0;
     auto take = [&](int64_t bytes) {
@@ -1161,16 +1176,21 @@
         off += (bytes + 255) / 256 * 256;
         return o;
     };
-    const int64_t o_pairs = take((int64_t)B * sizeof(KoptPair)), o_which = take((int64_t)(nc + 1) * 4);
+    const int64_t o_pairs = take((int64_t)B * sizeof(KoptPair)), o_which = take((int64_t)(nc + 1) * 4),
+                  o_todo = take((int64_t)(ntodo + 1) * 4), o_rowp = take((int64_t)B * 8), o_wrowp = take((int64_t)(nc + 1) * 8),
+                  o_sums = take((int64_t)B * 8);
     const int64_t table_bytes = off;
-    const int64_t o_sums = take((int64_t)B * 8), o_E = take((int64_t)B * FF * 8),
-                  o_SQ = take((int64_t)B * FF * 8), o_Z = take((int64_t)nc * F * Fh * 16), o_PW = take((int64_t)nc * FF * 8);
+    const int64_t o_E = take((int64_t)B * FF * 8), o_SQ = take((int64_t)B * FF * 8), o_Z = take((int64_t)nc * F * Fh * 16),
+                  o_PW = take((int64_t)nc * FF * 8);
     char* base = (char*)gd_scratch(ctx, off);
     if (!base) return GD_ERR_NOMEM;
     double* d_sums = (double*)(base + o_sums);
     KoptPair* d_pairs = (KoptPair*)(base + o_pairs);
     double* d_out = d_rows;
     int* d_which = (int*)(base + o_which);
+    const int* d_todo = (const int*)(base + o_todo);
+    const double* const* d_rowp = (const double* const*)(base + o_rowp);
+    const double* const* d_wrowp = (const double* const*)(base + o_wrowp);
     double* d_E = (double*)(base + o_E);
     double* d_SQ = (double*)(base + o_SQ);
     double2* d_Z = (double2*)(base + o_Z);
@@ -1179,10 +1199,17 @@
         std::vector<char> tab((size_t)table_bytes, 0);
         memcpy(tab.data() + o_pairs, hp.data(), (size_t)B * sizeof(KoptPair));
         if (nc) memcpy(tab.data() + o_which, which.data(), (size_t)nc * 4);
+        if (nc) memcpy(tab.data() + o_wrowp, wrows.data(), (size_t)nc * 8);
+        if (ntodo) memcpy(tab.data() + o_todo, todo.data(), (size_t)ntodo * 4);
+        memcpy(tab.data() + o_rowp, hrows.data(), (size_t)B * 8);
+        memcpy(tab.data() + o_sums, hsums.data(), (size_t)B * 8);
         GD_TRY(gd_stage_h2d(ctx, base, tab.data(), (size_t)table_bytes));
     }
-    k_hist_sums<<<B, 1024, 0, ctx->stream>>>(d_hist, (int)FF, d_sums);
-    GD_KERNEL_CHECK();
+    ctx->kopt_sums = d_sums, ctx->kopt_sums_count = B;
+    if (ntodo) {
+        k_hist_sums<<<ntodo, 1024, 0, ctx->stream>>>(d_rowp, d_todo, (int)FF, d_sums);
+        GD_KERNEL_CHECK();
+    }
     if (dct_fft) {
         const int RPB = F <= 256 ? 16 : (F <= 512 ? 8 : 4);
         const size_t lds = ((size_t)2 * F + (size_t)RPB * F) * 16;
@@ -1192,19 +1219,19 @@
         auto k1 = big ? k_dct_pass<1, true> : k_dct_pass<1, false>;
         GD_HIP(hipFuncSetAttribute((const void*)k0, hipFuncAttributeMaxDynamicSharedMemorySize, (int)lds));
         GD_HIP(hipFuncSetAttribute((const void*)k1, hipFuncAttributeMaxDynamicSharedMemorySize, (int)lds));
-        k0<<<grid, RPB * FT, lds, ctx->stream>>>(d_hist, F, plH, d_tw, d_ck, nullptr, d_E);
+        k0<<<grid, RPB * FT, lds, ctx->stream>>>(nullptr, F, plH, d_tw, d_ck, nullptr, d_E, d_rowp);
         GD_KERNEL_CHECK();
-        k1<<<grid, RPB * FT, lds, ctx->stream>>>(d_E, F, plH, d_tw, d_ck, d_sums, d_SQ);
+        k1<<<grid, RPB * FT, lds, ctx->stream>>>(d_E, F, plH, d_tw, d_ck, d_sums, d_SQ, nullptr);
         GD_KERNEL_CHECK();
     } else {
         const dim3 ggrid((F + 63) / 64, (F + 63) / 64, B);
-        k_gemm_nt<0><<<ggrid, 256, 0, ctx->stream>>>(D, 0, d_hist, FF, F, d_E, FF, nullptr);
+        k_gemm_nt<0><<<ggrid, 256, 0, ctx->stream>>>(D, 0, nullptr, FF, F, d_E, FF, nullptr, d_rowp);
         GD_KERNEL_CHECK();
         k_gemm_nt<1><<<ggrid, 256, 0, ctx->stream>>>(d_E, FF, D, 0, F, d_SQ, FF, d_sums);
         GD_KERNEL_CHECK();
     }
     if (nc > 0) {
-        k_gather_norm<<<dim3(64, nc), 256, 0, ctx->stream>>>(d_hist, d_which, d_sums, (int)FF, d_E);
+        k_gather_norm<<<dim3(64, nc), 256, 0, ctx->stream>>>(d_wrowp, d_which, d_sums, (int)FF, d_E);
         GD_KERNEL_CHECK();
         int rc = gd_fft_r2c_2d(ctx, F, F, nc, d_E, d_Z);
         if (rc) return rc;
@@ -1277,21 +1304,36 @@
     return gd_h2d(ctx, d_rows + (int64_t)B * KOPT_STRIDE, tab.data(), tab.size() * 8);
 }
 
-int gd_kopt2d(gd_ctx* ctx, int32_t B, int32_t F, const void* d_hist_v, const double* neff, const int32_t* do_corr,
-              const double* fallback_t, const double* corr, double* out) {
-    GD_REQUIRE(ctx && d_hist_v && neff && do_corr && fallback_t && corr && out && B > 0, "bad argument");
+int gd_kopt2d_src(gd_ctx* ctx, int32_t B, int32_t F, const void* d_hist_v, const void* const* row_ptrs, const double* known_sum,
+                  const double* neff, const int32_t* do_corr, const double* fallback_t, const double* corr, double* out) {
+    GD_REQUIRE(ctx && (d_hist_v || row_ptrs) && neff && do_corr && fallback_t && corr && out && B > 0, "bad argument");
     double* d_rows = (double*)gd_scratch2(ctx, (int64_t)B * KOPT_BLOCK_DOUBLES * 8);
     if (!d_rows) return GD_ERR_NOMEM;
     GD_TRY(kopt_upload_get_h_inputs(ctx, B, d_rows, neff, corr, do_corr));
-    GD_TRY(kopt_stage_a(ctx, B, F, d_hist_v, neff, do_corr, fallback_t, d_rows));
+    GD_TRY(kopt_stage_a(ctx, B, F, d_hist_v, row_ptrs, known_sum, neff, do_corr, fallback_t, d_rows));
     return kopt_stage_b(ctx, nullptr, B, d_rows, out);
 }
 
-int gd_kopt2d_enqueue(gd_ctx* ctx, int32_t B, int32_t F, const void* d_hist, const double* neff, const int32_t* do_corr,
-                      const double* fallback_t, const double* corr, void* d_rows, int32_t* ticket_out) {
+int gd_kopt2d(gd_ctx* ctx, int32_t B, int32_t F, const void* d_hist_v, const double* neff, const int32_t* do_corr,
+              const double* fallback_t, const double* corr, double* out) {
+    GD_REQUIRE(ctx && d_hist_v, "bad argument");
+    return gd_kopt2d_src(ctx, B, F, d_hist_v, nullptr, nullptr, neff, do_corr, fallback_t, corr, out);
+}
+
+int gd_kopt2d_sums(gd_ctx* ctx, int32_t B, double* sums_out) {
+    GD_REQUIRE(ctx && sums_out && B > 0 && ctx->kopt_sums && B == ctx->kopt_sums_count, "no optimiser launch of that size to read the sums of");
+    const char *lo = (const char*)ctx->scratch, *p = (const char*)ctx->kopt_sums;
+    GD_REQUIRE(lo && p >= lo && p + (int64_t)B * 8 <= lo + ctx->scratch_bytes, "the scratch block of that launch is gone");
+    GD_TRY(gd_fetch(ctx, sums_out, ctx->kopt_sums, (size_t)B * 8));
+    return gd_stream_sync(ctx);
+}
+
+int gd_kopt2d_enqueue_src(gd_ctx* ctx, int32_t B, int32_t F, const void* d_hist, const void* const* row_ptrs,
+                          const double* known_sum, const double* neff, const int32_t* do_corr, const double* fallback_t,
+                          const double* corr, void* d_rows, int32_t* ticket_out) {
     GD_REQUIRE(ctx && ticket_out && d_rows && neff && corr && do_corr && B > 0, "bad argument");
     GD_TRY(kopt_upload_get_h_inputs(ctx, B, (double*)d_rows, neff, corr, do_corr));
-    GD_TRY(kopt_stage_a(ctx, B, F, d_hist, neff, do_corr, fallback_t, (double*)d_rows));
+    GD_TRY(kopt_stage_a(ctx, B, F, d_hist, row_ptrs, known_sum, neff, do_corr, fallback_t, (double*)d_rows));
     const int slot = ctx->kopt_ev_next;
     ctx->kopt_ev_next = (slot + 1) % gd_ctx::kKoptEvents;
     if (!ctx->kopt_evs[slot]) GD_HIP(hipEventCreateWithFlags(&ctx->kopt_evs[slot], hipEventDisableTiming));
@@ -1300,6 +1342,12 @@
     return GD_OK;
 }
 
+int gd_kopt2d_enqueue(gd_ctx* ctx, int32_t B, int32_t F, const void* d_hist, const double* neff, const int32_t* do_corr,
+                      const double* fallback_t, const double* corr, void* d_rows, int32_t* ticket_out) {
+    GD_REQUIRE(ctx && d_hist, "bad argument");
+    return gd_kopt2d_enqueue_src(ctx, B, F, d_hist, nullptr, nullptr, neff, do_corr, fallback_t, corr, d_rows, ticket_out);
+}
+
 int gd_kopt2d_finish(gd_ctx* ctx, gd_ctx* stage_a_ctx, int32_t ticket, int32_t B, void* d_rows, double* out) {
     GD_REQUIRE(ctx && stage_a_ctx && ticket >= 0 && ticket < gd_ctx::kKoptEvents && stage_a_ctx->kopt_evs[ticket], "bad ticket");
     GD_HIP(hipSetDevice(ctx->device));
diff --git a/include/gdhip.h b/include/gdhip.h
--- a/include/gdhip.h
+++ b/include/gdhip.h
@@ -118,6 +118,12 @@
 int gd_kopt2d_enqueue(gd_ctx* ctx, int32_t B, int32_t F, const void* d_hist, const double* neff, const int32_t* do_corr,
                       const double* fallback_t, const double* corr, void* d_rows, int32_t* ticket_out);
 int gd_kopt2d_finish(gd_ctx* ctx, gd_ctx* stage_a_ctx, int32_t ticket, int32_t B, void* d_rows, double* out);
+int gd_kopt2d_src(gd_ctx* ctx, int32_t B, int32_t F, const void* d_hist, const void* const* row_ptrs, const double* known_sum,
+                  const double* neff, const int32_t* do_corr, const double* fallback_t, const double* corr, double* out);
+int gd_kopt2d_enqueue_src(gd_ctx* ctx, int32_t B, int32_t F, const void* d_hist, const void* const* row_ptrs,
+                          const double* known_sum, const double* neff, const int32_t* do_corr, const double* fallback_t,
+                          const double* corr, void* d_rows, int32_t* ticket_out);
+int gd_kopt2d_sums(gd_ctx* ctx, int32_t B, double* sums_out);
 int gd_get_h(gd_ctx* ctx, int32_t B, const double* psi, const double* neff, const double* corr, const int32_t* do_corr,
              double* out);
 
```
